# IuvenisSapiens/Qwen3-TTS-Rust

Hardware: AMD Instinct MI355X
Metric: audio-seconds generated per second (aggregate over GPUs) = concurrent real-time streams; RTF and first-chunk latency from the single-utterance leg (higher is better)
Workload: dtype i8

## Files before the change

### include/q3tts.h

```cpp
#ifndef Q3TTS_H
#define Q3TTS_H
#include <stdint.h>
#include <stddef.h>
#include "q3tts_spec.h"
#ifdef __cplusplus
extern "C" {
#endif

#define Q3TTS_OK 0
#define Q3TTS_ERR -1

const char* q3tts_last_error(void);
int q3tts_version(void);
int q3tts_device_count(void);

typedef struct q3tts_sampler_config {
    float temperature;
    int32_t top_k;
    float top_p;
    int32_t has_seed;
    uint64_t seed;
} q3tts_sampler_config;
void q3tts_sampler_config_default(q3tts_sampler_config* c);

// ... 309 lines not shown
                       uint16_t* ad);
int q3tts_op_matmul_float(const void* w , int32_t type, int32_t n, int32_t k, int32_t row0, int32_t nrows,
                          const float* x , int32_t ntok, float* y );
int q3tts_op_rmsnorm_quant(const float* x, const float* g, int32_t d, int32_t ntok, float eps, int8_t* xq, uint16_t* xd,
                           float* xn);
int q3tts_op_swiglu_quant(const float* gu, int32_t ff, int32_t ntok, int8_t* aq, uint16_t* ad);
int q3tts_op_argmax(const float* logits, int32_t n, int32_t start, int32_t end, int32_t mask_idx, int32_t* out);
int q3tts_op_sample(const float* logits, int32_t n, float temperature, int32_t top_k, float top_p, uint64_t seed, int32_t mask_idx,
                    int32_t n_draws, int32_t* out);
int q3tts_op_sample_rows(int32_t kernel, const float* logits, int32_t B, int32_t n, const float* temperature, const int32_t* top_k,
                         const float* top_p, const float* penalty, const uint64_t* seed, const int32_t* hist, const int32_t* hist_len,
                         int32_t hist_cap, int32_t n_draws, int32_t* out);
int q3tts_op_project(const float* x, const float* w , const float* b, int32_t n_in, int32_t n_out, float* y);
int q3tts_op_logprob_rows(const float* logits, int32_t B, int32_t n, int32_t stride, const int32_t* chosen, int32_t extra_idx,
                          float* out_chosen, float* out_extra);
int q3tts_op_score_rows(const float* tlogits, int32_t t_stride, const float* plogits, const int32_t* codes, int32_t F, float* out);
int q3tts_op_score_inputs(const float* hidden_proj, const float* const* tabs, const int64_t* tab_rows, int32_t dP, const int32_t* codes,
                          int32_t F, float* out);
int q3tts_op_kv_fork(uint16_t* k_cache, uint16_t* v_cache, int32_t n_pages, int32_t n_layer, int32_t n_kv, const int32_t* page_table,
                     int32_t n_seq, int32_t max_pages, int32_t src_seq, const int32_t* dst_seqs, int32_t n_dst, int32_t n_positions);
int q3tts_op_feedback_rows(const q3tts_assets* a, const int32_t* codes, int32_t n, const int32_t* trail_ids, int32_t n_trail, float* rows);
enum { Q3TTS_GEMM_AUTO = 0, Q3TTS_GEMM_SKINNY4 = 1, Q3TTS_GEMM_SKINNY8 = 2, Q3TTS_GEMM_SKINNY16 = 3,
       Q3TTS_GEMM_F32_1 = 4, Q3TTS_GEMM_F32_2 = 5,
       Q3TTS_GEMM_H1 = 6, Q3TTS_GEMM_H1_EPL = 7, Q3TTS_GEMM_H2 = 8, Q3TTS_GEMM_H2_EPL = 9,
       Q3TTS_GEMM_H3 = 10, Q3TTS_GEMM_H3_EPL = 11 };
enum { Q3TTS_EPI_NONE = 0, Q3TTS_EPI_GELU = 1, Q3TTS_EPI_RES_SCALE = 2 , Q3TTS_EPI_RES = 3 ,
       Q3TTS_EPI_SNAKE = 4  };
typedef struct q3tts_codec_gemm_desc {
    int32_t M, N, cin, taps, dil;
    const float* A; int64_t a_rows; int32_t lda, a_segT, a_skip;
    int32_t a_split, o_split;
    const float* W; const float* bias;
    int32_t epi; const float* res; int64_t res_floats; int32_t ldr, r_segT; int64_t r_skip;
    const float* scale; const float* snake_ea; const float* snake_ib;
    float* out; int64_t out_floats, out_off; int32_t ldo, o_segT; int64_t o_skip;
    int64_t ws_floats;
    int32_t form, ksplit, reducer;
    int32_t form_ran, ksplit_ran, reducer_ran;
} q3tts_codec_gemm_desc;
int q3tts_op_codec_gemm(q3tts_codec_gemm_desc* d);
int q3tts_codec_gemm_plan(q3tts_codec_gemm_desc* d);

enum { Q3TTS_CK_RVQ_SUM = 0, Q3TTS_CK_RMSNORM_ROWS = 1, Q3TTS_CK_LAYERNORM_ROWS = 2, Q3TTS_CK_ROPE_APPEND = 3, Q3TTS_CK_WINDOW_ATTN = 4,
       Q3TTS_CK_SWIGLU_ROWS = 5, Q3TTS_CK_DWCONV7 = 6, Q3TTS_CK_SNAKE = 7, Q3TTS_CK_SNAKE_SPLIT = 8, Q3TTS_CK_CONV_OUT_WAVE = 9,
       Q3TTS_CK_CONV_OUT_WIN = 10, Q3TTS_CK_HIST_LOAD = 11, Q3TTS_CK_HIST_SAVE = 12, Q3TTS_CK_HIST_ZERO = 13 };
typedef struct q3tts_codec_kernel_desc {
    int32_t kernel;
    int32_t G, T, C, H;
    int32_t n_heads, head_dim, window; float rope_base, eps, bias;
    const int64_t* meta;
    const int64_t* codes; int32_t n_q, cb_size;
    int32_t n_streams, stream;
    const float* in[3]; int64_t in_floats[3];
    const float* p0; const float* p1; int64_t p0_floats, p1_floats;
    float* out[3]; int64_t out_floats[3];
} q3tts_codec_kernel_desc;
int q3tts_op_codec_kernel(q3tts_codec_kernel_desc* d);

enum { Q3TTS_ATTN_AUTO = 0, Q3TTS_ATTN_UNFUSED = 1 , Q3TTS_ATTN_FUSED = 2 ,
       Q3TTS_ATTN_SHORT1 = 3, Q3TTS_ATTN_SHORT2 = 4 , Q3TTS_ATTN_GGML = 5  };
typedef struct q3tts_attention_desc {
    int32_t n_head, n_kv, n_layer, layer, ntok;
    const float* qkv; int32_t qkv_stride;
    const float* q_norm; const float* k_norm;
    float eps, rope_base; int32_t n_ctx; int32_t mrope_sec[4];
    const int32_t* seq; const int32_t* slot; const int32_t* pos; int32_t uniform_pos;
    const int32_t* page_table; int32_t n_seq, max_pages;
    uint16_t* k_cache; uint16_t* v_cache; int32_t n_pages;
    int32_t fused, fused_max_tok, same_seq, short_attn_min, hpw1_max, float_mode, ggml_mode;
    int32_t form;
    float* att; int8_t* aq; uint16_t* ad;
    int32_t form_ran;
} q3tts_attention_desc;
int q3tts_op_attention(q3tts_attention_desc* d);
int q3tts_op_attention_keyed(q3tts_attention_desc* d, const uint64_t* keys, int32_t key_stride, int32_t qkv_rows);
int q3tts_attention_plan(q3tts_attention_desc* d);

enum { Q3TTS_LOP_GEMV = 0, Q3TTS_LOP_GATEUP = 1, Q3TTS_LOP_NORM = 2, Q3TTS_LOP_NORM_GEMV = 3, Q3TTS_LOP_NORM_ARGMAX = 4, Q3TTS_LOP_NORM_GATEUP = 5,
       Q3TTS_LOP_F_GEMV = 6, Q3TTS_LOP_F_GATEUP = 7 };
enum { Q3TTS_LIN_AUTO = 0, Q3TTS_LIN_GEMV_Q8 = 1, Q3TTS_LIN_GEMM_Q8_TOK = 2, Q3TTS_LIN_GEMM_Q8_MFMA = 3, Q3TTS_LIN_GEMM_Q8_TILE1 = 4,
       Q3TTS_LIN_GEMV_KQ = 5, Q3TTS_LIN_GEMM_KQ_MFMA = 6, Q3TTS_LIN_GU_Q8_TILE1 = 7, Q3TTS_LIN_GU_Q8_MFMA = 8, Q3TTS_LIN_GU_KQ_MFMA = 9,
       Q3TTS_LIN_GU_UNFUSED = 10, Q3TTS_LIN_NORM = 11, Q3TTS_LIN_NORM_WG = 12, Q3TTS_LIN_GEMV_NORM = 13, Q3TTS_LIN_GEMV_NORM_ARGMAX = 14,
       Q3TTS_LIN_GU_SWIGLU_NORM = 15, Q3TTS_LIN_F_GEMV = 16, Q3TTS_LIN_F_MFMA16 = 17, Q3TTS_LIN_F_MFMA = 18, Q3TTS_LIN_F_GU_MFMA16 = 19,
       Q3TTS_LIN_F_GU_UNFUSED = 20 };
typedef struct q3tts_linear_desc {
    int32_t op, form;
    int32_t nw; const void* raw[3]; int32_t type[3]; int32_t rows[3]; int32_t kq_layout;
    int32_t K, row0, nrows, nrows_valid, ntok, ff;
    int32_t lpr, mt, ztiles;
    int32_t fused;
    const int8_t* xq; const uint16_t* xd; int32_t a_rows;
    const float* x; int64_t x_floats; int32_t x_off, x_stride;
    const float* h_in; int64_t h_floats; int32_t h_stride;
    const uint64_t* idx_keys; const int32_t* idx; int32_t idx_stride;
    const float* parts; int64_t parts_floats; int32_t nparts, parts_stride; int64_t parts_slab;
    const float* g; float eps;
    float* h_out; float* xn_out;
    int8_t* xq_out; uint16_t* xd_out;
    uint64_t* keys; int64_t n_keys; int32_t key_stride; const int32_t* mask_per_tok; int32_t idx_add;
    float* out; int64_t out_floats, out_off; int32_t out_stride;
    int8_t* aq; uint16_t* ad;
    int32_t form_ran, lpr_ran, mt_ran, z_ran;
} q3tts_linear_desc;
int q3tts_op_linear(q3tts_linear_desc* d);
int q3tts_linear_plan(q3tts_linear_desc* d);
uint64_t q3tts_argmax_key(float v, int32_t idx);

enum { Q3TTS_SEL_SAMPLE = 0, Q3TTS_SEL_SAMPLE_PRED = 1, Q3TTS_SEL_ARGMAX = 2, Q3TTS_SEL_ARGMAX_KEYS = 3 };
#define Q3TTS_SELECT_SENTINEL 0xA5C3F00D5A3C0FF1ull
typedef struct q3tts_select_desc {
    int32_t kernel;
    int32_t B, n, stride, row_off;
    const float* logits;
    const float* temperature; const int32_t* top_k; const float* top_p;
    const int32_t* mask_idx;
    const uint64_t* seed;
    const uint32_t* draw0;
    int32_t n_draws;
    const float* penalty; const int32_t* hist; const int32_t* hist_len; int32_t hist_cap; const int32_t* cur_code;
    int32_t out_stride;
    int32_t start, end, add;
    int32_t* tokens;
    uint64_t* out_raw;
    uint32_t* draws_out;
} q3tts_select_desc;
int q3tts_op_select_rows(q3tts_select_desc* d);

enum { Q3TTS_GLUE_PROJECT_MT = 0, Q3TTS_GLUE_PROJECT_TABLE = 1, Q3TTS_GLUE_FEEDBACK_KEYS = 2, Q3TTS_GLUE_GATHER_ROWS_KEYS = 3,
       Q3TTS_GLUE_ADVANCE_KEYS = 4, Q3TTS_GLUE_STALL_SAVE = 5, Q3TTS_GLUE_ADVANCE_KEYS_GATED = 6 };
#define Q3TTS_GLUE_GUARD 64
typedef struct q3tts_guarded { void* p; int64_t n; } q3tts_guarded;
typedef struct q3tts_frame_glue_desc {
    int32_t kernel;
    int32_t ntok;
    int32_t n_in, n_out, x_stride, x_off, out_stride;
    const float* x; int64_t x_floats;
    const float* w; const float* b;
    const float* const* tables; const int64_t* table_rows;
    int32_t row_len, key_stride;
    const float* tts_pad;
    int32_t trail; const int32_t* trail_ids; int32_t ids_stride; const float* text_table; int64_t text_rows;
    const int32_t* n_trail; const int32_t* open; const int32_t* max_frames;
    int32_t hist_stride;
    q3tts_guarded out;
    q3tts_guarded keys, next_key0;
    q3tts_guarded finished, n_frames, t_slot, t_pos, hist;
    q3tts_guarded hidden, save_hidden;
    q3tts_guarded draws, pdraws, save_draws;
} q3tts_frame_glue_desc;
int q3tts_op_frame_glue(q3tts_frame_glue_desc* d);

int q3tts_pcm_out_plan(int32_t rate, int32_t* L, int32_t* M, int32_t* n_taps, int32_t* taps_per_phase);
int64_t q3tts_pcm_out_filter(int32_t rate, float* h32, int64_t cap);
int64_t q3tts_pcm_out_samples(int32_t rate, int64_t n_native);
int q3tts_pcm_format_check(const q3tts_pcm_format* f);
int q3tts_op_pcm_convert(const float* in, int32_t G, const int32_t* chunk_samples, int32_t n_chunks, const int32_t* streams, int32_t n_streams,
                         const q3tts_pcm_format* fmt, const int32_t* reset_before, void* const* out, const int64_t* out_bytes, int64_t* n_out,
                         float* hist_store);

int64_t q3tts_tsm_samples(int32_t rate_pct, int64_t n_native, int32_t final);
int q3tts_tsm_windows(float* w, float* w2);
int q3tts_op_tsm(const float* in, int32_t G, const int32_t* chunk_samples, int32_t n_chunks, const int32_t* streams, int32_t n_streams,
                 const int32_t* rate_pct, const int32_t* encoding, const int32_t* reset_before, int32_t flush, void* const* out,
                 const int64_t* out_bytes, int64_t* n_out, int32_t* const* delta_trace, const int64_t* trace_len, float* hist_store);

#ifdef __cplusplus
}
// ... 3 lines not shown
```

### qwen3-tts-rust_amd/csrc/capi_ops.cpp

```cpp
#include "../../include/q3tts.h"
#include "transformer.h"
#include "host_logic.h"
#include "kdev.h"
#include "codec.h"
#include "kernels.h"
#include "pcm_out.h"
#include "tsm.h"

using namespace q3;
#define Q3_API_BEGIN try {
#define Q3_API_END(failval) } catch (const std::exception& ex) { set_last_error(ex.what()); return failval; } catch (...) { set_last_error("unknown error"); return failval; }
static void require_gpu() {
    int n = 0;
    if (hipGetDeviceCount(&n) != hipSuccess || n <= 0) throw Error("no HIP device available: the HIP path is the only compute path (no CPU fallback)");
}

static int attention_op_plan(const q3tts_attention_desc& d) {
    AttnPlanIn a;
    a.ntok = d.ntok; a.fused = d.fused != 0; a.fused_max_tok = d.fused_max_tok; a.same_seq = d.same_seq != 0; a.short_attn_min = d.short_attn_min;
    a.n_head = d.n_head; a.n_kv = d.n_kv; a.hpw1_max = d.hpw1_max > 0 ? d.hpw1_max : short_attn_hpw1_max();
    a.float_mode = d.float_mode != 0; a.ggml_mode = d.ggml_mode != 0;
    return plan_attention(a);
}

// ... 43 lines not shown
        }
        dkeys.alloc((size_t)(nt - 1) * key_stride + 1); dkeys.upload((const q3_u64*)keys, dkeys.n);
    }
    DevBuf<float> qkv((size_t)(keys ? qkv_rows : nt) * qs); qkv.upload(d.qkv, qkv.n);
    const QkvRows rows(qkv.p, qs, dkeys.p, key_stride);
    DevBuf<float> qn(128), kn(128); qn.upload(d.q_norm, 128); kn.upload(d.k_norm, 128);
    std::vector<float> hc, hs;
    build_rope_tables(d.rope_base, d.n_ctx, hc, hs);
    DevBuf<float> rc(hc.size()), rs(hs.size()); rc.upload(hc.data(), hc.size()); rs.upload(hs.data(), hs.size());
    DevBuf<int32_t> sec(4); sec.upload(d.mrope_sec, 4);
    DevBuf<int32_t> dseq, dslot, dpos, dtab;
    TokMeta tm{nullptr, nullptr, nullptr};
    if (d.uniform_pos >= 0) tm.uniform_pos = d.uniform_pos;
    else {
        dseq.alloc(nt); dseq.upload(d.seq, nt); dslot.alloc(nt); dslot.upload(d.slot, nt); dpos.alloc((size_t)nt * 4); dpos.upload(d.pos, (size_t)nt * 4);
        tm.seq = dseq.p; tm.slot = dslot.p; tm.pos = dpos.p;
    }
    const size_t cache_halfs = (size_t)d.n_pages * d.n_layer * d.n_kv * 8192;
    DevBuf<uint16_t> kc(cache_halfs), vc(cache_halfs);
    kc.upload(d.k_cache, cache_halfs); vc.upload(d.v_cache, cache_halfs);
    KvCache kv;
    kv.k = kc.p; kv.v = vc.p; kv.page_table = nullptr; kv.max_pages = d.page_table ? d.max_pages : 1; kv.n_layer = d.n_layer; kv.n_kv = d.n_kv;
    if (d.page_table) { dtab.alloc((size_t)d.n_seq * d.max_pages); dtab.upload(d.page_table, dtab.n); kv.page_table = dtab.p; }
    DevBuf<float> att((size_t)nt * dq), qrot, scores;
    DevBuf<int8_t> aq((size_t)nt * dq); DevBuf<uint16_t> ad((size_t)nt * (dq / 32));
    switch (form) {
    case ATTN_UNFUSED:
        qrot.alloc((size_t)nt * dq);
        launch_qk_rope_append(0, rows, nullptr, d.n_head, d.n_kv, qn.p, kn.p, d.eps, rc.p, rs.p, d.n_ctx, sec.p, tm, kv, d.layer, qrot.p, nt);
        launch_attention(0, qrot.p, d.n_head, d.n_kv, tm, kv, d.layer, att.p, aq.p, ad.p, nt);
        break;
    case ATTN_FUSED:
        launch_attention_fused(0, rows, d.n_head, d.n_kv, qn.p, kn.p, d.eps, rc.p, rs.p, d.n_ctx, sec.p, tm, kv, d.layer, aq.p, ad.p, nt);
        break;
    case ATTN_SHORT1: case ATTN_SHORT2:
        launch_attention_short(0, form == ATTN_SHORT1 ? 1 : 2, rows, d.n_head, d.n_kv, qn.p, kn.p, d.eps, rc.p, rs.p, d.n_ctx, sec.p, tm, kv,
                               d.layer, aq.p, ad.p, nt, att.p);
        break;
    default:
        scores.alloc((size_t)nt * d.n_head * d.n_ctx);
        gg_qk_rope_append(0, qkv.p, qs, d.n_head, d.n_kv, qn.p, kn.p, d.eps, rc.p, rs.p, d.n_ctx, sec.p, tm, kv, d.layer, nt);
        gg_attention(0, qkv.p, qs, d.n_head, d.n_kv, tm, kv, d.layer, att.p, scores.p, d.n_ctx, nt);
        break;
    }
    Q3_LAUNCH_CHECK();
    Q3_HIP(hipDeviceSynchronize());
    kc.download(d.k_cache, cache_halfs); vc.download(d.v_cache, cache_halfs);
    if (d.att && form != ATTN_FUSED) att.download(d.att, att.n);
    if (form != ATTN_GGML) { aq.download(d.aq, aq.n); ad.download(d.ad, ad.n); }
    if (keys) qkv.download(const_cast<float*>(d.qkv), qkv.n);
    d.form_ran = form;
}

static bool lin_quant(const q3tts_linear_desc& d) { return d.op <= LOP_NORM_GATEUP && d.op != LOP_NORM; }
static bool lin_kq(const q3tts_linear_desc& d) {
    if (d.kq_layout || d.nw > 1) return true;
    return d.type[0] != Q3_T_Q8_0;
}
static int lin_rows(const q3tts_linear_desc& d) { int n = 0; for (int i = 0; i < d.nw; i++) n += d.rows[i]; return n; }
static int lin_wts(const q3tts_linear_desc& d) {
    if (d.op >= LOP_F_GEMV) return d.type[0];
    if (!lin_kq(d)) return 0;
    int n = 0, last = -1;
    for (int i = 0; i < d.nw; i++) if (d.type[i] != last) { n++; last = d.type[i]; }
    return n == 1 ? d.type[0] : -1;
}
static LinearPlanIn lin_plan_in(const q3tts_linear_desc& d) {
    LinearPlanIn in;
    in.op = d.op; in.K = d.K; in.row0 = d.row0; in.nrows = d.nrows; in.ntok = d.ntok; in.ff = d.ff;
    in.kq = lin_quant(d) && lin_kq(d); in.wts = lin_wts(d); in.has_wt = true;
    if (in.kq) { int n = 0, last = -1; for (int i = 0; i < d.nw; i++) if (d.type[i] != last) { n++; last = d.type[i]; } in.kq_parts = n; }
    in.out_stride = d.out_stride; in.out_addr = (uintptr_t)d.out_off * 4 + (d.out ? (uintptr_t)d.out : 0);
    in.x_stride = d.x_stride; in.x_addr = (uintptr_t)d.x_off * 4 + (d.x ? (uintptr_t)d.x : 0);
    in.aq_addr = 0; in.fused = d.fused != 0;
    return in;
}
static LinearPlan lin_plan(const q3tts_linear_desc& d) {
    Q3_CHECK(d.op >= LOP_GEMV && d.op <= LOP_F_GATEUP, "unknown linear op");
    Q3_CHECK(d.K >= 256 && d.K % 256 == 0 && d.ntok >= 1 && d.ntok <= 65535 && d.nrows >= 1 && d.row0 >= 0, "bad linear shape");
    return plan_linear(lin_plan_in(d));
}
static bool in_set(int v, std::initializer_list<int> s) { for (int x : s) if (v == x) return true; return false; }
static int op_of_form(int f) {
    if (f <= LIN_GEMM_KQ_MFMA) return LOP_GEMV;
    if (f <= LIN_GU_UNFUSED) return LOP_GATEUP;
    if (f <= LIN_NORM_WG) return LOP_NORM;
    if (f == LIN_GEMV_NORM) return LOP_NORM_GEMV;
    if (f == LIN_GEMV_NORM_ARGMAX) return LOP_NORM_ARGMAX;
    if (f == LIN_GU_SWIGLU_NORM) return LOP_NORM_GATEUP;
    if (f <= LIN_F_MFMA) return LOP_F_GEMV;
    return LOP_F_GATEUP;
}
static void lin_check(const q3tts_linear_desc& d, const LinearPlan& p) {
    const int f = p.form, K = d.K, nt = d.ntok, ntiles = (nt + 31) / 32;
    Q3_CHECK(f >= LIN_GEMV_Q8 && f <= LIN_F_GU_UNFUSED && op_of_form(f) == d.op, "the form does not compute this op");
    const bool quant = lin_quant(d), kq = quant && lin_kq(d), norm = d.op >= LOP_NORM && d.op <= LOP_NORM_GATEUP;
    if (d.op != LOP_NORM) {
        Q3_CHECK(d.nw >= 1 && d.nw <= 3, "1 to 3 weight tensors");
        for (int i = 0; i < d.nw; i++) Q3_CHECK(d.raw[i] && d.rows[i] >= 1, "missing weight tensor");
        if (d.op >= LOP_F_GEMV) Q3_CHECK(d.nw == 1 && (d.type[0] == Q3_T_F32 || d.type[0] == Q3_T_F16 || d.type[0] == Q3_T_BF16), "float ops take one f32 / f16 / bf16 tensor");
        else if (kq) for (int i = 0; i < d.nw; i++) Q3_CHECK(in_set(d.type[i], {Q3_T_Q8_0, Q3_T_Q5_K, Q3_T_Q6_K}) && d.rows[i] % 32 == 0, "K-quant layout: Q8_0 / Q5_K / Q6_K tensors of 32-row multiples");
        Q3_CHECK(d.row0 + d.nrows <= lin_rows(d), "rows past the matrix");
    }
    if (d.op == LOP_GATEUP) Q3_CHECK(K <= 2048, "int8 gate/up: K <= 2048 (k_swiglu_quant reads one super-segment slab)");
    if (d.op == LOP_GATEUP || d.op == LOP_NORM_GATEUP || d.op == LOP_F_GATEUP)
        Q3_CHECK(d.row0 == 0 && d.nrows == 2 * d.ff && d.ff >= 1 && d.ff % (d.op == LOP_F_GATEUP ? 1 : 32) == 0, "gate/up: row0 0, nrows 2 * ff, ff % 32 == 0");
    if (quant && !norm) Q3_CHECK(d.xq && d.xd && d.a_rows >= nt, "int8 activations [a_rows >= ntok][K]");
    if (d.op >= LOP_F_GEMV) Q3_CHECK(d.x && d.x_off >= 0 && d.x_stride >= K && d.x_off + (int64_t)(nt - 1) * d.x_stride + K <= d.x_floats, "float activations out of their buffer");
    if (norm) {
        Q3_CHECK(K <= 2048 && d.h_in && d.g && d.h_stride >= K, "norm prologue: K <= 2048, h_in and g required");
        Q3_CHECK(!(d.idx && d.idx_keys), "idx or idx_keys, not both");
        if (d.idx) Q3_CHECK(f == LIN_NORM, "int32 row indices: NORM only");
        for (int t = 0; t < nt; t++) {
            int64_t row = t;
            if (d.idx) row = d.idx[(size_t)t * d.idx_stride];
            else if (d.idx_keys) row = key_code(d.idx_keys[(size_t)t * d.idx_stride]);
            Q3_CHECK(row >= 0 && row * d.h_stride + K <= d.h_floats, "selected h_in row outside h_in");
        }
        Q3_CHECK(d.nparts >= 0 && (d.nparts == 0 || (d.parts && d.parts_stride >= K && d.parts_slab >= 0 &&
                 (int64_t)(d.nparts - 1) * d.parts_slab + (int64_t)(nt - 1) * d.parts_stride + K <= d.parts_floats)), "residual slabs out of their buffer");
        if (f == LIN_NORM && d.nparts > 1) Q3_CHECK(d.parts_slab == (int64_t)nt * d.parts_stride, "NORM: slabs are ntok * parts_stride apart");
        if (d.op == LOP_NORM) Q3_CHECK(d.xq_out && d.xd_out, "NORM: xq_out / xd_out required");
    }
    if (in_set(d.op, {LOP_GEMV, LOP_NORM_GEMV, LOP_F_GEMV, LOP_F_GATEUP})) {
        const int64_t cols = d.op == LOP_F_GATEUP ? d.ff : d.nrows;
        const int64_t slabs = d.op == LOP_GEMV ? (K / 256 + 7) / 8 : 1;
        Q3_CHECK(d.out && d.out_off >= 0 && d.out_stride >= cols && d.out_off + (slabs * nt - 1) * d.out_stride + cols <= d.out_floats, "output out of its buffer");
    }
    if (in_set(d.op, {LOP_GATEUP, LOP_NORM_GATEUP})) Q3_CHECK(d.aq && d.ad, "gate/up: aq / ad required");
    if (f == LIN_GEMV_NORM_ARGMAX) {
        Q3_CHECK(d.keys && d.key_stride >= 1 && (int64_t)(nt - 1) * d.key_stride < d.n_keys, "argmax keys out of their buffer");
        Q3_CHECK(d.nrows_valid >= 1 && d.nrows_valid <= d.nrows, "1 <= nrows_valid <= nrows");
    }
    const bool q8 = quant && !kq;
    switch (f) {
    case LIN_GEMV_Q8: case LIN_GEMV_KQ:
        Q3_CHECK(f == LIN_GEMV_Q8 ? q8 : kq, "GEMV_Q8 takes the Q8_0 layout, GEMV_KQ the K-quant layout");
        Q3_CHECK(in_set(p.lpr, {2, 4, 8}) && in_set(p.mt, {1, 2, 4, 8}), "lpr in {2,4,8}, mt in {1,2,4,8}");
        break;
    case LIN_GEMM_Q8_TOK: Q3_CHECK(q8, "GEMM_Q8_TOK takes the Q8_0 layout"); break;
    case LIN_GEMM_Q8_MFMA: case LIN_GEMM_KQ_MFMA:
        Q3_CHECK(f == LIN_GEMM_Q8_MFMA ? q8 : kq, "GEMM_Q8_MFMA takes the Q8_0 layout, GEMM_KQ_MFMA the K-quant layout");
        Q3_CHECK(p.z >= 1 && p.z <= ntiles, "1 <= ztiles <= token tiles");
        break;
    case LIN_GEMM_Q8_TILE1:
        Q3_CHECK(q8 && K <= 1024 && d.nrows % 4 == 0 && d.out_stride % 4 == 0 && ((uintptr_t)(d.out + d.out_off) & 15) == 0 && p.z == ntiles,
                 "GEMM_Q8_TILE1: Q8_0, K <= 1024, nrows % 4 == 0, out_stride % 4 == 0, 16-byte out, ztiles == token tiles");
        break;
    case LIN_GU_Q8_TILE1: case LIN_GU_Q8_MFMA: case LIN_GU_KQ_MFMA:
        Q3_CHECK(f == LIN_GU_KQ_MFMA ? (kq && lin_wts(d) != -1) : q8, "GU_Q8_*: Q8_0 layout; GU_KQ_MFMA: K-quant layout of one tensor type");
        Q3_CHECK((K == 1024 || K == 2048) && d.ff % 32 == 0, "fused gate/up: K in {1024, 2048}, ff % 32 == 0");
        Q3_CHECK(p.z >= (ntiles + 3) / 4 && p.z <= ntiles && (f != LIN_GU_Q8_TILE1 || p.z == ntiles), "fused gate/up: ceil(tiles/4) <= ztiles <= tiles (TILE1: == tiles)");
        break;
    case LIN_GEMV_NORM: case LIN_GEMV_NORM_ARGMAX: case LIN_GU_SWIGLU_NORM:
        Q3_CHECK(f == LIN_GU_SWIGLU_NORM ? (in_set(p.mt, {1, 2, 4}) && lin_wts(d) != -1) : in_set(p.mt, {1, 2, 4, 8}), "mt out of range / GU_SWIGLU_NORM needs one tensor type");
        Q3_CHECK(f == LIN_GU_SWIGLU_NORM || (f == LIN_GEMV_NORM_ARGMAX ? p.lpr == 2 : in_set(p.lpr, {2, 4, 8})), "GEMV_NORM: lpr in {2,4,8}; ARGMAX: lpr 2");
        break;
    case LIN_F_GEMV: Q3_CHECK(in_set(p.mt, {1, 2, 4, 8}), "mt in {1,2,4,8}"); break;
    case LIN_F_MFMA16: case LIN_F_MFMA: case LIN_F_GU_MFMA16:
        Q3_CHECK(d.row0 % 64 == 0 && ((uintptr_t)(d.x + d.x_off) & 15) == 0 && d.x_stride % 4 == 0, "float matrix-core forms: row0 % 64 == 0, 16-byte x, x_stride % 4 == 0");
        if (f == LIN_F_GU_MFMA16) Q3_CHECK(d.ff % 16 == 0, "F_GU_MFMA16: ff % 16 == 0");
        break;
    default: break;
    }
}
static void lin_run(q3tts_linear_desc* dp) {
    Q3_CHECK(dp, "null linear descriptor");
    q3tts_linear_desc& d = *dp;
    LinearPlan p = lin_plan(d);
    if (d.form != LIN_AUTO) {
        Q3_CHECK(d.form >= LIN_GEMV_Q8 && d.form <= LIN_F_GU_UNFUSED, "unknown linear form");
        LinearPlan fp; fp.form = d.form; fp.nseg = d.K / 256;
        const int f = d.form, ntiles = (d.ntok + 31) / 32;
        const int mt_def = d.ntok == 1 ? 1 : d.ntok == 2 ? 2 : d.ntok <= 4 ? 4 : 8;
        fp.mt = d.mt ? d.mt : (p.form == f && p.mt ? p.mt : (f == LIN_GU_SWIGLU_NORM ? (mt_def > 4 ? 4 : mt_def) : mt_def));
        fp.lpr = d.lpr ? d.lpr : (p.form == f && p.lpr ? p.lpr : (f == LIN_GEMV_NORM_ARGMAX ? 2 : 8));
        int zdef = p.form == f && p.z ? p.z : ntiles;
        fp.z = d.ztiles ? d.ztiles : zdef;
        p = fp;
    }
    lin_check(d, p);
    const int K = d.K, nt = d.ntok, ff = d.ff;
    DevBuf<uint8_t> storage, fw, fwt;
    Q8Mat m; FMat fm;
    if (d.op >= LOP_F_GEMV) {
        const int n = d.rows[0];
        const size_t esz = d.type[0] == Q3_T_F32 ? 4 : 2;
        fw.alloc((size_t)n * K * esz); fw.upload((const uint8_t*)d.raw[0], fw.n);
        fwt.alloc((size_t)((n + 63) / 64) * 64 * K * esz);
        launch_tile_float(0, fw.p, fwt.p, d.type[0], n, K);
        fm.w = fw.p; fm.wt = fwt.p; fm.type = d.type[0]; fm.N = n; fm.K = K;
    } else if (d.op != LOP_NORM) {
        m = lin_kq(d) ? kqmat_from_host(d.raw, d.type, d.rows, d.nw, K, storage) : q8mat_from_host(d.raw[0], d.rows[0], K, storage);
    }
    DevBuf<int8_t> dxq; DevBuf<uint16_t> dxd; DevBuf<float> dx, dh, dparts, dg, dhout, dxn, dout, dgu;
    DevBuf<q3_u64> dkeys_in, dkeys; DevBuf<int32_t> didx, dmask; DevBuf<int8_t> daq, dxq_out; DevBuf<uint16_t> dad, dxd_out;
    if (d.xq) { dxq.alloc((size_t)d.a_rows * K); dxq.upload(d.xq, dxq.n); dxd.alloc((size_t)d.a_rows * (K / 32)); dxd.upload(d.xd, dxd.n); }
    if (d.op >= LOP_F_GEMV) { dx.alloc((size_t)d.x_floats); dx.upload(d.x, dx.n); }
    NormPro a{};
    const bool norm = d.op >= LOP_NORM && d.op <= LOP_NORM_GATEUP;
    if (norm) {
        dh.alloc((size_t)d.h_floats); dh.upload(d.h_in, dh.n);
        dg.alloc(K); dg.upload(d.g, K);
        a.h_in = dh.p; a.h_stride = d.h_stride; a.g = dg.p; a.eps = d.eps; a.idx_stride = d.idx_stride;
        if (d.idx_keys) { dkeys_in.alloc((size_t)(nt - 1) * d.idx_stride + 1); dkeys_in.upload((const q3_u64*)d.idx_keys, dkeys_in.n); a.idx_keys = dkeys_in.p; }
        if (d.idx) { didx.alloc((size_t)(nt - 1) * d.idx_stride + 1); didx.upload(d.idx, didx.n); }
        if (d.nparts > 0) { dparts.alloc((size_t)d.parts_floats); dparts.upload(d.parts, dparts.n); }
        a.parts = dparts.p; a.nparts = d.nparts; a.parts_stride = d.parts_stride; a.parts_slab = (size_t)d.parts_slab;
        if (d.h_out) { dhout.alloc((size_t)nt * K); dhout.upload(d.h_out, dhout.n); a.h_out = dhout.p; }
        if (d.xn_out) { dxn.alloc((size_t)nt * K); dxn.upload(d.xn_out, dxn.n); a.xn_out = dxn.p; }
    }
    if (d.out) { dout.alloc((size_t)d.out_floats); dout.upload(d.out, dout.n); }
    if (d.aq) { daq.alloc((size_t)nt * ff); daq.upload(d.aq, daq.n); dad.alloc((size_t)nt * (ff / 32)); dad.upload(d.ad, dad.n); }
    float* out = d.out ? dout.p + d.out_off : nullptr;
    switch (p.form) {
    case LIN_GEMV_Q8: case LIN_GEMM_Q8_TOK: case LIN_GEMM_Q8_MFMA: case LIN_GEMM_Q8_TILE1: case LIN_GEMV_KQ: case LIN_GEMM_KQ_MFMA:
        run_gemv_q8(0, p, m, d.row0, d.nrows, dxq.p, dxd.p, out, d.out_stride, nt);
        break;
    case LIN_GU_Q8_TILE1: case LIN_GU_Q8_MFMA: case LIN_GU_KQ_MFMA:
        run_gateup_q8(0, p, m, ff, dxq.p, dxd.p, daq.p, dad.p, nt);
        break;
    case LIN_GU_UNFUSED: {
        dgu.alloc((size_t)((K / 256 + 7) / 8) * nt * 2 * ff);
        LinearPlanIn gi = linear_plan_in(LOP_GEMV, m, 0, 2 * ff, nt);
        gi.out_stride = 2 * ff; gi.out_addr = (uintptr_t)dgu.p;
        const LinearPlan gp = plan_linear(gi);
        run_gemv_q8(0, gp, m, 0, 2 * ff, dxq.p, dxd.p, dgu.p, 2 * ff, nt);
        launch_swiglu_quant(0, dgu.p, ff, daq.p, dad.p, nt);
        p.lpr = gp.lpr; p.mt = gp.mt; p.z = gp.z;
        break;
    }
    case LIN_NORM: {
        dxq_out.alloc((size_t)nt * K); dxq_out.upload(d.xq_out, dxq_out.n); dxd_out.alloc((size_t)nt * (K / 32)); dxd_out.upload(d.xd_out, dxd_out.n);
        launch_rmsnorm_quant(0, norm_args(a, K, dxq_out.p, dxd_out.p, didx.p), nt);
        break;
    }
    case LIN_NORM_WG:
        dxq_out.alloc((size_t)nt * K); dxq_out.upload(d.xq_out, dxq_out.n); dxd_out.alloc((size_t)nt * (K / 32)); dxd_out.upload(d.xd_out, dxd_out.n);
        launch_rmsnorm_quant_wg(0, a, K, dxq_out.p, dxd_out.p, nt);
        break;
    case LIN_GEMV_NORM: case LIN_GEMV_NORM_ARGMAX: {
        ArgmaxEpi am{};
        if (p.form == LIN_GEMV_NORM_ARGMAX) {
            dkeys.alloc((size_t)d.n_keys); dkeys.upload((const q3_u64*)d.keys, dkeys.n);
            if (d.mask_per_tok) { dmask.alloc(nt); dmask.upload(d.mask_per_tok, nt); }
            am.keys = dkeys.p; am.key_stride = d.key_stride; am.mask_per_tok = dmask.p; am.idx_add = d.idx_add;
            run_gemv_q8_norm(0, p, m, d.row0, d.nrows_valid, a, nullptr, 0, nt, &am);
        } else run_gemv_q8_norm(0, p, m, d.row0, d.nrows, a, out, d.out_stride, nt, nullptr);
        break;
    }
    case LIN_GU_SWIGLU_NORM: run_gateup_swiglu(0, p, m, ff, a, daq.p, dad.p, nt); break;
    case LIN_F_GEMV: case LIN_F_MFMA16: case LIN_F_MFMA:
        run_gemv_float(0, p, fm, d.row0, d.nrows, dx.p + d.x_off, d.x_stride, out, d.out_stride, nt);
        break;
    case LIN_F_GU_MFMA16:
        dgu.alloc((size_t)nt * ff);
        run_gateup_float(0, p, fm, ff, dx.p + d.x_off, d.x_stride, dgu.p, nt);
        break;
    case LIN_F_GU_UNFUSED: {
        dgu.alloc((size_t)nt * 2 * ff);
        LinearPlanIn gi = lin_plan_in(d); gi.op = LOP_F_GEMV;
        const LinearPlan gp = plan_linear(gi);
        run_gemv_float(0, gp, fm, 0, 2 * ff, dx.p + d.x_off, d.x_stride, dgu.p, 2 * ff, nt);
        DevBuf<float> act((size_t)nt * ff);
        launch_swiglu_f32(0, dgu.p, ff, act.p, nt);
        Q3_HIP(hipMemcpy2D(out, (size_t)d.out_stride * 4, act.p, (size_t)ff * 4, (size_t)ff * 4, nt, hipMemcpyDeviceToDevice));
        Q3_HIP(hipDeviceSynchronize());
        p.lpr = gp.lpr; p.mt = gp.mt; p.z = gp.z;
        break;
    }
    default: throw Error("unhandled linear form");
    }
    Q3_LAUNCH_CHECK();
    if (p.form == LIN_F_GU_MFMA16) Q3_HIP(hipMemcpy2D(out, (size_t)d.out_stride * 4, dgu.p, (size_t)ff * 4, (size_t)ff * 4, nt, hipMemcpyDeviceToDevice));
    Q3_HIP(hipDeviceSynchronize());
    if (d.out) dout.download(d.out, dout.n);
    if (d.aq) { daq.download(d.aq, daq.n); dad.download(d.ad, dad.n); }
    if (d.h_out) dhout.download(d.h_out, dhout.n);
    if (d.xn_out) dxn.download(d.xn_out, dxn.n);
    if (dxq_out.p) { dxq_out.download(d.xq_out, dxq_out.n); dxd_out.download(d.xd_out, dxd_out.n); }
    if (dkeys.p) dkeys.download((q3_u64*)d.keys, dkeys.n);
    d.form_ran = p.form; d.lpr_ran = p.lpr; d.mt_ran = p.mt; d.z_ran = p.z;
}

template <class T> struct GlueBuf {
    DevBuf<T> d; T* host = nullptr; size_t n = 0;
    void up(const q3tts_guarded& g, size_t core, const char* what) {
        Q3_CHECK(g.p && g.n >= (int64_t)(core + 2 * Q3TTS_GLUE_GUARD), std::string("guarded buffer too small or missing: ") + what);
        host = (T*)g.p; n = (size_t)g.n;
        d.alloc(n); d.upload(host, n);
    }
    T* p() const { return d.p + Q3TTS_GLUE_GUARD; }
    void down() { if (host) d.download(host, n); }
};

extern "C" {

int q3tts_op_attention(q3tts_attention_desc* d) {
    Q3_API_BEGIN
    require_gpu();
    attention_op_run(d);
    return Q3TTS_OK;
    Q3_API_END(Q3TTS_ERR)
}

int q3tts_op_attention_keyed(q3tts_attention_desc* d, const uint64_t* keys, int32_t key_stride, int32_t qkv_rows) {
    Q3_API_BEGIN
    require_gpu();
    Q3_CHECK(keys, "null keys");
    attention_op_run(d, keys, key_stride, qkv_rows);
    return Q3TTS_OK;
    Q3_API_END(Q3TTS_ERR)
}

int q3tts_attention_plan(q3tts_attention_desc* d) {
    Q3_API_BEGIN
    Q3_CHECK(d && d->ntok >= 1 && d->n_kv >= 1 && d->n_head >= 1, "bad attention shape");
    d->form_ran = attention_op_plan(*d);
    return Q3TTS_OK;
    Q3_API_END(Q3TTS_ERR)
}

int q3tts_op_linear(q3tts_linear_desc* d) {
    Q3_API_BEGIN
    require_gpu();
    lin_run(d);
    return Q3TTS_OK;
    Q3_API_END(Q3TTS_ERR)
}

int q3tts_linear_plan(q3tts_linear_desc* d) {
    Q3_API_BEGIN
    Q3_CHECK(d, "null linear descriptor");
    const LinearPlan p = lin_plan(*d);
    d->form_ran = p.form; d->lpr_ran = p.lpr; d->mt_ran = p.mt; d->z_ran = p.z;
    return Q3TTS_OK;
    Q3_API_END(Q3TTS_ERR)
}

uint64_t q3tts_argmax_key(float v, int32_t idx) { return pack_key(v, idx); }

int q3tts_op_kv_fork(uint16_t* k_cache, uint16_t* v_cache, int32_t n_pages, int32_t n_layer, int32_t n_kv, const int32_t* page_table,
                     int32_t n_seq, int32_t max_pages, int32_t src_seq, const int32_t* dst_seqs, int32_t n_dst, int32_t n_positions) {
    Q3_API_BEGIN
    Q3_CHECK(k_cache && v_cache && page_table && dst_seqs, "null argument");
    Q3_CHECK(n_pages >= 1 && n_layer >= 1 && n_kv >= 1 && n_seq >= 1 && max_pages >= 1, "bad cache / page table shape");
    Q3_CHECK((int64_t)n_layer * n_kv <= 65536 && (int64_t)n_pages * n_layer * n_kv <= ((int64_t)1 << 24), "cache too large for the test surface");
    Q3_CHECK(n_dst >= 1, "n_dst must be >= 1");
    Q3_CHECK(n_positions >= 1 && (int64_t)n_positions <= (int64_t)max_pages * 64, "n_positions must be in [1, max_pages * 64]");
    Q3_CHECK(src_seq >= 0 && src_seq < n_seq, "source sequence out of range");
    const int np = (n_positions + 63) / 64;
    std::vector<int> owner((size_t)n_pages, -1);
    std::vector<char> listed((size_t)n_seq, 0);
    listed[src_seq] = 1;
    for (int d = -1; d < n_dst; d++) {
        const int seq = d < 0 ? src_seq : dst_seqs[d];
        if (d >= 0) {
            Q3_CHECK(seq >= 0 && seq < n_seq, "destination sequence out of range");
            Q3_CHECK(seq != src_seq, "a destination equals the source");
            Q3_CHECK(!listed[seq], "a destination is listed twice");
// ... 939 lines not shown
```

### qwen3-tts-rust_amd/csrc/engine.cpp

```cpp
#include "engine.h"
#include "../../include/q3tts.h"
#include <algorithm>
#include <cmath>
#include <chrono>
#include "kdev.h"
#include <functional>

namespace q3 {

static std::string quant_dir(const std::string& q) {
    if (q == "q5_k_m") return "gguf_q5_k_m";
    if (q == "q8_0") return "gguf_q8_0";
    if (q == "bf16") return "gguf_bf16";
    if (q == "f16") return "gguf_f16";
    return "gguf";
}
static double now_ms() {
    return std::chrono::duration<double, std::milli>(std::chrono::steady_clock::now().time_since_epoch()).count();
}

Engine::Engine(const EngineParams& p) : p_(p) {
    Q3_CHECK(p.max_batch >= 1 && p.max_batch <= 512, "max_batch out of range");
    Q3_HIP(hipGetDevice(&dev_));
    Q3_HIP(hipStreamCreateWithFlags(&st_, hipStreamNonBlocking));
    const std::string dir = p.model_dir + "/" + quant_dir(p.quant);
    assets_.reset(new HostAssets(dir + "/qwen3_assets.gguf"));
    const int B = p.max_batch;
    B_ = B;
    talker_.reset(new Transformer(dir + "/qwen3_tts_talker.gguf", Q3_TALKER_NCTX, std::max(256, B)));
    predictor_.reset(new Transformer(dir + "/qwen3_tts_predictor.gguf", Q3_PRED_NCTX, 2 * B));
    if (const char* e = std::getenv("Q3_PRED_FUSED_MAX")) predictor_->set_fused_max_tokens(atoi(e));
    {
        int min_tok = 8;
        if (const char* e = std::getenv("Q3_SHORT_ATTN_MIN")) min_tok = atoi(e);
        predictor_->set_short_attention(min_tok, 17);
    }
    Q3_CHECK(talker_->hp().n_embd == Q3_EMBD, "talker n_embd must be 2048 (reference hard-codes 2048-wide rows)");
    dP_ = predictor_->hp().n_embd;
    Q3_CHECK(assets_->proj_out == dP_ && assets_->proj_in == Q3_EMBD, "proj shape does not match predictor n_embd");
    Q3_CHECK(assets_->n_codec == 16, "need 16 codec embedding tables");
    Q3_CHECK(predictor_->hp().n_vocab >= 15 * Q3_CODEBOOK_SIZE, "predictor vocab < 15*2048");
    Q3_CHECK(dP_ % 16 == 0, "projection width must be a multiple of 16");
    {
        const std::vector<float> wt = project_wt(assets_->proj_w, Q3_EMBD, dP_), wb = project_wblk(assets_->proj_w, Q3_EMBD, dP_);
        d_proj_wt_.alloc(wt.size()); d_proj_wt_.upload(wt.data(), wt.size());
        d_proj_wblk_.alloc(wb.size()); d_proj_wblk_.upload(wb.data(), wb.size());
    }
    d_proj_b_.alloc(dP_); d_proj_b_.upload(assets_->proj_b, dP_);
    d_tts_pad_.alloc(Q3_EMBD); d_tts_pad_.upload(assets_->tts_pad(), Q3_EMBD);
    std::vector<const float*> ptrs(16);
    std::vector<int64_t> rows(16);
    for (int q = 0; q < 16; q++) {
        const size_t n = (size_t)assets_->codec_rows[q] * Q3_EMBD;
        d_codec_tab_[q].alloc(n); d_codec_tab_[q].upload(assets_->codec[q], n);
        d_proj_tab_[q].alloc((size_t)assets_->codec_rows[q] * dP_);
        launch_project_table(st_, d_codec_tab_[q].p, assets_->codec_rows[q], d_proj_wt_.p, d_proj_b_.p, Q3_EMBD, dP_, d_proj_tab_[q].p);
        ptrs[q] = d_codec_tab_[q].p; rows[q] = assets_->codec_rows[q];
    }
    d_tab_ptrs_.alloc(16); d_tab_ptrs_.upload(ptrs.data(), 16);
    d_tab_rows_.alloc(16); d_tab_rows_.upload(rows.data(), 16);
    pred_l0_table_ = !predictor_->ggml_mode();
    if (const char* e = std::getenv("Q3_PRED_L0_TABLE")) if (e[0] == '0') pred_l0_table_ = false;
    if (pred_l0_table_) {
        const int qs = (predictor_->hp().n_head + 2 * predictor_->hp().n_kv) * 128;
        Transformer wide(*predictor_, 256);
        for (int q = 1; q < 15; q++) {
            d_qkv0_tab_[q].alloc((size_t)assets_->codec_rows[q] * qs);
            wide.build_layer0_qkv(st_, d_proj_tab_[q].p, dP_, assets_->codec_rows[q], d_qkv0_tab_[q].p);
            pred_table_bytes_ += d_qkv0_tab_[q].n * sizeof(float);
        }
        Q3_HIP(hipStreamSynchronize(st_));
    }
    const int pages_per_seq = (p.max_prompt + p.max_steps + 1 + 63) / 64;
    kv_rows_ = (int64_t)pages_per_seq * 64;
    kv_t_.reset(new KvPool(talker_->hp().n_layer, talker_->hp().n_kv, B * pages_per_seq + 1, B + 1, pages_per_seq));
    kv_p_.reset(new KvPool(predictor_->hp().n_layer, predictor_->hp().n_kv, B, B, 1));
    for (int b = 0; b < B; b++) kv_p_->ensure(b, 16);
    pred_identity_pages_ = true;
    for (int b = 0; b < B; b++) if (kv_p_->page(b, 0) != b) pred_identity_pages_ = false;
    if (const char* e = std::getenv("Q3_UNIFORM_META")) if (e[0] == '0') pred_identity_pages_ = false;
    kv_t_->ensure(B, 1);
    {
        const char* e = std::getenv("Q3_ASYNC_PREFILL");
        async_pf_ = B > 1 && !(e && e[0] == '0');
    }
    if (async_pf_) {
        talker_pf_.reset(new Transformer(*talker_, 256));
        Q3_HIP(hipStreamCreateWithFlags(&st_pf_, hipStreamNonBlocking));
        Q3_HIP(hipEventCreate(&pf_done_)); Q3_HIP(hipEventCreate(&pf_e0_));
        lane_alloc(pf_, talker_pf_.get(), st_pf_, 256, true, (size_t)4096 * (Q3_EMBD * 4 + 24 + 68 + 64) + ((size_t)1 << 16) + (size_t)B * 4);
    }
    hist_stride_ = p.max_steps * 16;
    tl_stride_ = (Q3_SAMPLE_END + 31) & ~31;
    slots_ = SlotTable(B); d_slots_.alloc(slots_.host.size()); slots_.dev = d_slots_.p;
    d_keys_.alloc(16 * B); d_next_key0_.alloc(B); d_hist_.alloc((size_t)B * hist_stride_);
    d_rngkey_.alloc((size_t)8 * B); d_draws_.alloc(B); d_prngkey_.alloc((size_t)8 * B); d_pdraws_.alloc(B);
    d_rngkey_.zero(); d_draws_.zero(); d_prngkey_.zero(); d_pdraws_.zero(); d_plogits_.alloc((size_t)B * Q3_CODEBOOK_SIZE);
    d_tlogits_.alloc((size_t)B * tl_stride_); d_thidden_.alloc((size_t)B * Q3_EMBD); d_pin_.alloc((size_t)2 * B * dP_);
    d_fb_.alloc((size_t)B * Q3_EMBD);
    d_hist_.zero(); d_tlogits_.zero(); d_thidden_.zero();
    std::vector<int32_t> seq(B), slot((size_t)16 * B), pos((size_t)16 * B * 4);
    for (int b = 0; b < B; b++) {
        seq[b] = b;
        for (int i = 0; i < 16; i++) { slot[(size_t)i * B + b] = i; for (int s = 0; s < 4; s++) pos[((size_t)i * B + b) * 4 + s] = i; }
    }
    d_pseq_.alloc(B); d_pseq_.upload(seq.data(), B);
    d_pslot_.alloc(slot.size()); d_pslot_.upload(slot.data(), slot.size());
    d_ppos_.alloc(pos.size()); d_ppos_.upload(pos.data(), pos.size());
    h_pend_.assign(B, std::vector<int32_t>()); h_pend_off_.assign(B, 0);
    slot_req_.assign(B, nullptr);
    if (const char* e = std::getenv("Q3_SCORE_WIDTH")) score_w_ = std::max(16, std::min(64, atoi(e)));
    if (async_pf_) { d_pf_logits_.alloc((size_t)B * tl_stride_); d_pf_hidden_.alloc((size_t)B * Q3_EMBD); }
    {
        std::vector<q3_u64> k0((size_t)16 * B, pack_key(-INFINITY, 0)), n0(B, pack_key(-INFINITY, 0));
        d_keys_.upload(k0.data(), k0.size()); d_next_key0_.upload(n0.data(), n0.size());
    }
    lane_alloc(ar_, talker_.get(), st_, talker_->max_tok(), false, (size_t)talker_->max_tok() * Q3_EMBD * 4 + (size_t)B * 4096 + ((size_t)1 << 20));
    Q3_HIP(hipDeviceSynchronize());
    upload_slot_state();
    if (p.load_codec) {
        Q3_CHECK(p.max_steps <= Q3TTS_CODEC_MAX_FRAMES, "max_steps above Q3TTS_CODEC_MAX_FRAMES: a request's codec stream could not be decoded to its end");
        static const int group_env = [] { const char* e = std::getenv("Q3_CODEC_GROUP"); return e ? atoi(e) : 0; }();
        const int group_cap = group_env > 0 ? group_env : (B >= 128 ? 32 : 16);
        const int n_cs = B + std::min(B, 16), gmax = std::max(1, std::min(B, group_cap));
        static const int lanes_env = [] { const char* e = std::getenv("Q3_CODEC_LANES"); return e ? atoi(e) : 0; }();
        const int n_lanes = B > 1 ? (lanes_env > 0 ? std::min(lanes_env, 8) : 2) : 1;
        codec_.reset(new CodecDecoder(p.model_dir + "/onnx/q3tts_codec.gguf", n_cs, 4, n_lanes, gmax));
        st2_.resize(n_lanes);
        for (auto& s2 : st2_) Q3_HIP(hipStreamCreateWithFlags(&s2, hipStreamNonBlocking));
        slot_cap_ = (size_t)p.max_steps * codec_->samples_per_frame();
        Q3_HIP(hipHostMalloc((void**)&pcm_pinned_, (size_t)n_cs * slot_cap_ * sizeof(float)));
        Q3_HIP(hipHostMalloc((void**)&pre_tails_, (size_t)Q3TTS_MAX_PREAMBLES * Q3_PCM_HIST * sizeof(float)));
        for (int i = Q3TTS_MAX_PREAMBLES - 1; i >= 0; i--) pre_tail_free_.push_back(i);
        for (int c = n_cs - 1; c >= 0; c--) cs_free_.push_back(c);
        decode_w_ = q3::decode_width(n_cs, B);
    }
    Q3_HIP(hipStreamSynchronize(st_));
    Q3_HIP(hipDeviceSynchronize());
    ar_.cur.reset();
}

void Engine::lane_alloc(PrefillLane& L, Transformer* talker, hipStream_t st, int chunk, bool async, size_t arena_bytes) {
    L.talker = talker; L.st = st; L.chunk = chunk; L.async = async;
    L.d_rows.alloc((size_t)chunk * Q3_EMBD); L.d_seq.alloc(chunk); L.d_slot.alloc(chunk); L.d_pos.alloc(4 * (size_t)chunk);
    L.d_codes.alloc((size_t)chunk * 16); L.d_ids.alloc(chunk); L.d_fork_dst.alloc(B_);
    L.cur.cap = arena_bytes;
    Q3_HIP(hipHostMalloc((void**)&L.arena, arena_bytes));
}
void* Engine::stage_take(PrefillLane& L, size_t bytes) {
    size_t at = L.cur.take(bytes);
    if (at == StageCursor::NONE) {
        Q3_CHECK(!L.async, "prefill staging arena overflow");
        Q3_HIP(hipStreamSynchronize(L.st));
        L.cur.reset();
        at = L.cur.take(bytes);
        Q3_CHECK(at != StageCursor::NONE, "staging request larger than the arena");
    }
    return L.arena + at;
}
void Engine::h2d(void* dst, const void* src, size_t bytes) {
    void* p = stage_alloc(bytes);
    std::memcpy(p, src, bytes);
    Q3_HIP(hipMemcpyAsync(dst, p, bytes, hipMemcpyHostToDevice, st_));
}
void* Engine::d2h_begin(const void* src, size_t bytes) {
    void* p = stage_alloc(bytes);
    Q3_HIP(hipMemcpyAsync(p, src, bytes, hipMemcpyDeviceToHost, st_));
    return p;
}

struct CandSet { std::vector<float> prompt; std::vector<int32_t> trail; };
struct Engine::Req {
    int64_t id = 0;
// ... 851 lines not shown
    q3_u64 armed[17]; std::fill_n(armed, 17, pack_key(-INFINITY, 0));
    bool prefix_pcm = false;
    for (Req* r : batch) prefix_pcm = prefix_pcm || (r->want_pcm && r->r.n_prefix >= 4);
    {
        DecHold hold(this, codec_ != nullptr && prefix_pcm);
        for (Req* r : batch) {
            const int b = r->slot;
            slots_.load(b, r->r);
            const int k = r->r.n_prefix;
            const uint32_t draws = r->r.sampler.temperature > 0.0f ? (uint32_t)k : 0u, pdraws = 15u * (uint32_t)k;
            if (k > 0) {
                h2d(d_hist_.p + (size_t)b * hist_stride_, r->prefix_own.data(), (size_t)k * 64);
                push_frames(*r->chunker, r->prefix_own.data(), k);
            }
            StdRng rng(r->seed);
            h2d(d_rngkey_.p + (size_t)b * 8, rng.key(), 32);
            h2d(d_draws_.p + b, &draws, 4);
            if (r->r.opts.pred_sampled()) {
                StdRng prng(r->seed ^ (uint64_t)Q3_PRED_SEED_XOR);
                h2d(d_prngkey_.p + (size_t)b * 8, prng.key(), 32);
                h2d(d_pdraws_.p + b, &pdraws, 4);
            }
            h_pend_[b].clear();
            std::vector<int32_t> ids;
            { std::lock_guard<std::mutex> lk(mu_); ids = r->trail_ids(); slots_.hi(SF_OPEN)[b] = r->r.open && !r->closed; }
            slots_.hi(SF_NTRAIL)[b] = (int)ids.size();
            if (!ids.empty()) h2d(d_trail_.p + (size_t)b * p_.max_prompt, ids.data(), ids.size() * 4);
            h2d(d_keys_.p + (size_t)b * 16, armed, 16 * 8);
            h2d(d_next_key0_.p + b, armed, 8);
            if (lp_ready_.load()) {
                const int32_t rec = r->r.logprobs ? 1 : 0;
                h2d(d_lp_rec_.p + b, &rec, 4);
                if (rec) Q3_HIP(hipMemsetD32Async((hipDeviceptr_t)(d_lp_.p + (size_t)b * lp_rows_ * Q3_LOGPROB_COLS), (int)q3_f32_bits(Q3_LOGPROB_NONE),
                                                  (size_t)lp_rows_ * Q3_LOGPROB_COLS, st_));
            }
            slots_.live[b] = 1;
        }
    }
    upload_slot_state();
}

void Engine::activate() {
    std::vector<Req*> batch, dropped, scores;
    batch.swap(pf_batch_);
    {
        std::lock_guard<std::mutex> lk(mu_);
        const double t = now_ms();
        for (Req* r : batch) if (r->cancel) { r->prefill_ms = t - r->t_submit; dropped.push_back(r); }
        batch.erase(std::remove_if(batch.begin(), batch.end(), [](Req* r) { return r->cancel; }), batch.end());
    }
    for (Req* r : dropped) retire(r, false);
    for (Req* r : batch) if (r->score) scores.push_back(r);
    batch.erase(std::remove_if(batch.begin(), batch.end(), [](Req* r) { return r->score; }), batch.end());
    go_live(batch);
    for (Req* r : batch) {
        const int b = r->slot;
        Q3_HIP(hipMemcpyAsync(d_thidden_.p + (size_t)b * Q3_EMBD, d_pf_hidden_.p + (size_t)b * Q3_EMBD, (size_t)Q3_EMBD * 4, hipMemcpyDeviceToDevice, st_));
        SampleArgs sa = first_head_args(d_pf_logits_.p + (size_t)b * tl_stride_, b);
        if (resumed_penalised(r->r)) head_history(sa, b);
        launch_sample(st_, sa, 1);
        if (r->r.logprobs) first_head_logprobs(st_, d_pf_logits_.p + (size_t)b * tl_stride_, b, r->r.n_prefix);
    }
    Q3_HIP(hipStreamSynchronize(st_));
    { float ms = 0; Q3_HIP(hipEventElapsedTime(&ms, pf_e0_, pf_done_)); stats.prefill_ms += ms; }
    n_prefilling_ = 0;
    {
        const double t = now_ms();
        std::lock_guard<std::mutex> lk(mu_);
        for (Req* r : batch) r->prefill_ms = t - r->t_submit;
        for (Req* r : scores) r->prefill_ms = t - r->t_submit;
        n_active_ += (int)batch.size();
    }
    finish_scores(scores);
}

void Engine::ensure_score() {
    std::lock_guard<std::mutex> lk(sc_mu_);
    if (sc_ready_.load()) return;
    std::lock_guard<std::mutex> cap(capture_mutex());
    int prev = 0;
    Q3_HIP(hipGetDevice(&prev));
    Q3_HIP(hipSetDevice(dev_));
    try {
        const int W = score_w_, rows = std::max(talker_->max_tok(), 256);
        pred_sc_.reset(new Transformer(*predictor_, 16 * W));
        kv_sc_.reset(new KvPool(predictor_->hp().n_layer, predictor_->hp().n_kv, W, W, 1));
        for (int w = 0; w < W; w++) kv_sc_->ensure(w, 16);
        std::vector<int32_t> seq, slot, pos;
        for (int F = 1; F <= W; F++)
            for (int p = 0; p < 16; p++)
                for (int f = 0; f < F; f++) { seq.push_back(f); slot.push_back(p); for (int s4 = 0; s4 < 4; s4++) pos.push_back(p); }
        d_sc_seq_.alloc(seq.size()); d_sc_seq_.upload(seq.data(), seq.size());
        d_sc_slot_.alloc(slot.size()); d_sc_slot_.upload(slot.data(), slot.size());
        d_sc_pos_.alloc(pos.size()); d_sc_pos_.upload(pos.data(), pos.size());
        std::vector<const float*> tabs(15); std::vector<int64_t> tab_rows(15);
        for (int q = 0; q < 15; q++) { tabs[q] = d_proj_tab_[q].p; tab_rows[q] = assets_->codec_rows[q]; }
        d_sc_tabs_.alloc(15); d_sc_tabs_.upload(tabs.data(), 15);
        d_sc_tab_rows_.alloc(15); d_sc_tab_rows_.upload(tab_rows.data(), 15);
        d_sc_codes_.alloc((size_t)rows * 16); d_sc_tlogits_.alloc((size_t)rows * tl_stride_); d_sc_hidden_.alloc((size_t)rows * Q3_EMBD);
        d_sc_hproj_.alloc((size_t)W * dP_); d_sc_in_.alloc((size_t)16 * W * dP_); d_sc_plogits_.alloc((size_t)15 * W * Q3_CODEBOOK_SIZE);
        d_sc_out_.alloc((size_t)B_ * p_.max_steps * Q3_LOGPROB_COLS);
        Q3_HIP(hipStreamSynchronize(nullptr));
    } catch (...) { (void)hipSetDevice(prev); throw; }
    Q3_HIP(hipSetDevice(prev));
    sc_ready_ = true;
}

int64_t Engine::submit_score(const float* prompt, int n_prompt, const int32_t* trail, int n_trail, const int32_t* codes, int n) {
    if (const char* why = score_refusal(prompt, n_prompt, p_.max_prompt, trail, n_trail, codes, n, p_.max_steps, kv_rows_, talker_->ggml_mode()))
        throw Error(why);
    ensure_score();
    if (n_trail > 0) ensure_text_stream();
    std::unique_ptr<Req> r(new Req());
    r->score = true;
    GenRequest& g = r->r;
    g.n_prompt = n_prompt; g.max_steps = n; g.sampler.temperature = 0.0f; g.n_trail = n_trail;
    g.n_prefix = n - 1;
    r->prompt_own.assign(prompt, prompt + (size_t)n_prompt * Q3_EMBD); g.prompt = r->prompt_own.data();
    r->trail_own.assign(trail, trail + n_trail); g.trail = r->trail_own.data();
    r->prefix_own.assign(codes, codes + (size_t)n * 16); g.prefix = r->prefix_own.data();
    r->t_submit = now_ms();
    std::lock_guard<std::mutex> lk(mu_);
    return enqueue(std::move(r), pending_);
}

void Engine::score_chunk(hipStream_t st, Transformer& talker, const std::vector<Req*>& batch, const std::vector<ScoreRun>& runs, int32_t* h_codes) {
    if (runs.empty()) return;
    const int W = score_w_;
    int at = 0;
    for (const ScoreRun& run : runs) {
        Req* r = batch[run.req];
        Q3_CHECK((size_t)(at + run.n) * 16 <= d_sc_codes_.n && run.frame + run.n <= r->r.max_steps, "score rows outside the chunk buffers");
        std::copy(r->prefix_own.begin() + (size_t)run.frame * 16, r->prefix_own.begin() + (size_t)(run.frame + run.n) * 16, h_codes + (size_t)at * 16);
        Q3_HIP(hipMemcpyAsync(d_sc_codes_.p + (size_t)at * 16, h_codes + (size_t)at * 16, (size_t)run.n * 64, hipMemcpyHostToDevice, st));
        talker.head(st, run.row, run.n, 0, tl_stride_, d_sc_tlogits_.p + (size_t)at * tl_stride_, tl_stride_, nullptr, -1, d_sc_hidden_.p + (size_t)at * Q3_EMBD);
        for (int f0 = 0; f0 < run.n; f0 += W) {
            const int F = std::min(W, run.n - f0);
            const int32_t* codes = d_sc_codes_.p + (size_t)(at + f0) * 16;
            launch_project_blk(st, d_sc_hidden_.p + (size_t)(at + f0) * Q3_EMBD, Q3_EMBD, d_proj_wblk_.p, d_proj_b_.p, Q3_EMBD, dP_, d_sc_hproj_.p, dP_, F);
            launch_score_inputs(st, d_sc_hproj_.p, d_sc_tabs_.p, d_sc_tab_rows_.p, dP_, codes, F, d_sc_in_.p);
            const size_t m0 = (size_t)16 * F * (F - 1) / 2;
            TokMeta tm{d_sc_seq_.p + m0, d_sc_slot_.p + m0, d_sc_pos_.p + m0 * 4};
            Transformer::Input in; in.x = d_sc_in_.p; in.x_stride = dP_;
            pred_sc_->set_same_seq_tokens(true);
            pred_sc_->forward(st, in, 16 * F, tm, kv_sc_->view(), nullptr);
            for (int q = 0; q < 15; q++)
                pred_sc_->head(st, (q + 1) * F, F, q * Q3_CODEBOOK_SIZE, Q3_CODEBOOK_SIZE, d_sc_plogits_.p + (size_t)q * W * Q3_CODEBOOK_SIZE, Q3_CODEBOOK_SIZE);
            ScoreRowsArgs sa;
            sa.tlogits = d_sc_tlogits_.p + (size_t)(at + f0) * tl_stride_; sa.t_stride = tl_stride_;
            sa.plogits = d_sc_plogits_.p; sa.p_head_stride = (size_t)W * Q3_CODEBOOK_SIZE; sa.codes = codes;
            sa.out = d_sc_out_.p + ((size_t)r->slot * p_.max_steps + run.frame + f0) * Q3_LOGPROB_COLS;
            launch_score_rows(st, sa, F);
        }
        at += run.n;
    }
    Q3_LAUNCH_CHECK();
}

void Engine::finish_scores(const std::vector<Req*>& scores) {
    for (Req* r : scores) {
        const int b = r->slot, n = r->r.max_steps;
        bool cancelled;
        { std::lock_guard<std::mutex> lk(mu_); cancelled = r->cancel; }
        const float* rows = nullptr;
        if (!cancelled) {
            ar_.cur.reset();
            rows = (const float*)d2h_begin(d_sc_out_.p + (size_t)b * p_.max_steps * Q3_LOGPROB_COLS, (size_t)n * Q3_LOGPROB_COLS * 4);
// ... 451 lines not shown
```

### qwen3-tts-rust_amd/csrc/engine.h

```cpp
#pragma once
#include "transformer.h"
#include "host_logic.h"
#include "sched_logic.h"
#include "codec.h"
#include <atomic>
#include <condition_variable>
#include <deque>
#include <map>
#include <memory>
#include <mutex>
#include <thread>

namespace q3 {

struct EngineParams {
    std::string model_dir;
    std::string quant = "q8_0";
    int max_batch = 1;
    int max_prompt = 1024;
    int max_steps = Q3_DEFAULT_MAX_STEPS;
    bool load_codec = true;
    bool use_graph = true;
};

// ... 75 lines not shown
    int register_voice(const Voice& v);
    const Voice& voice(int id) const;

    const HostAssets& assets() const { return *assets_; }
    Transformer& talker() { return *talker_; }
    Transformer& predictor() { return *predictor_; }
    CodecDecoder* codec() { return codec_.get(); }
    EngineStats stats; void reset_stats() { stats = EngineStats(); }
    void set_instrument(bool on) { instrument_ = on; }
    size_t bytes_per_frame_step(int batch, double mean_ctx) const;
    size_t pred_table_bytes() const { return pred_table_bytes_; }
    hipStream_t stream() const { return st_; }
    int max_batch() const { return B_; }
    int device() const { return dev_; }

private:
    struct Req;
    struct FrameGraph {
        int width = 0; hipGraph_t graph = nullptr; hipGraphExec_t exec = nullptr;
        DevBuf<int32_t> seqA, slotA, posA;
    };
    void record_frame(FrameGraph& fg, FrameVariant v);
    FrameGraph& frame_graph(int width, FrameVariant v, bool capture);
    void validate(const GenRequest& g) const;
    void ensure_text_stream();
    Req& req(int64_t id);
    int64_t enqueue(std::unique_ptr<Req> r, std::deque<Req*>& queue);
    struct PrefillLane {
        Transformer* talker = nullptr; hipStream_t st = nullptr; int chunk = 0; bool async = false;
        DevBuf<float> d_rows; DevBuf<int32_t> d_seq, d_slot, d_pos;
        DevBuf<int32_t> d_codes, d_ids, d_fork_dst;
        unsigned char* arena = nullptr; StageCursor cur;
    };
    void lane_alloc(PrefillLane& L, Transformer* talker, hipStream_t st, int chunk, bool async, size_t arena_bytes);
    void* stage_take(PrefillLane& L, size_t bytes);
    void prefill_wave(PrefillLane& L, const std::vector<Req*>& wave, bool sampled);
    void head_live(Req* lead, const std::vector<Req*>& rest, int tok, bool sampled);
    void head_staged(Req* lead, const std::vector<Req*>& rest, int tok);
    SampleArgs first_head_args(const float* logits_row, int b) const;
    void feedback_rows(hipStream_t st, const std::vector<Req*>& batch, const std::vector<FbRun>& fb, int32_t* hc, int32_t* d_codes, int32_t* d_ids, float* d_rows);
    void head_history(SampleArgs& sa, int b) const;
    static bool resumed_penalised(const GenRequest& g) { return g.n_prefix > 0 && g.opts.penalised(); }
    void first_head_logprobs(hipStream_t st, const float* logits_row, int b, int row);
    void ensure_score();
    void score_chunk(hipStream_t st, Transformer& talker, const std::vector<Req*>& batch, const std::vector<ScoreRun>& runs, int32_t* h_codes);
    void finish_scores(const std::vector<Req*>& scores);
    static void split_sets(const std::vector<Req*>& batch, std::vector<Req*>& lead, std::vector<std::vector<Req*>>& rest);
    void fork_sets(hipStream_t st, const std::vector<Req*>& lead, const std::vector<std::vector<Req*>>& rest, int32_t* h_dst, int32_t* d_dst);
    static int kv_positions(const GenRequest& g, bool score) { return score ? g.n_prompt + g.n_prefix + 1 : g.n_prompt + g.max_steps + 1; }
    void prefill_async(const std::vector<Req*>& wave);
    void go_live(const std::vector<Req*>& batch);
    void activate();
    void admit_decodes();
    void enqueue_decodes();
    void admit(bool stalled);
    void run_group();
    void collect_appends();
    void collect_cancels();
    void harvest(bool block);
    void purge_chunks(Req* r);
    void retire(Req* r, bool flush_tail);
    void decoder_main();
    int64_t copy_pcm(const Req& r, void* out, int64_t off, int64_t cap) const;
    static int64_t pack_fmt(const q3tts_pcm_format& f) { return (int64_t)f.sample_rate * 4 + f.encoding; }
    static q3tts_pcm_format unpack_fmt(int64_t v) { return q3tts_pcm_format{(int32_t)(v / 4), (int32_t)(v % 4)}; }
    std::atomic<int64_t> out_fmt_{(int64_t)Q3_PCM_NATIVE_RATE * 4 + Q3_PCM_F32};
    std::atomic<int> rate_pct_{100};
    void take_rate(Req* r, int max_steps, int given = -1) const;
    void upload_slot_state();
    void* stage_alloc(size_t bytes) { return stage_take(ar_, bytes); }
    void h2d(void* dst, const void* src, size_t bytes);
    void* d2h_begin(const void* src, size_t bytes);

    EngineParams p_;
    hipStream_t st_ = nullptr; int dev_ = 0;
    std::vector<hipStream_t> st2_;
    float* pcm_pinned_ = nullptr; size_t slot_cap_ = 0;
    unsigned char* pcm_stage(const Req& r, size_t add) const;
    std::unique_ptr<HostAssets> assets_;
    std::unique_ptr<Transformer> talker_, predictor_, talker_pf_;
    hipStream_t st_pf_ = nullptr; PrefillLane ar_, pf_;
    DevBuf<float> d_pf_logits_, d_pf_hidden_;
    std::vector<Req*> pf_batch_; hipEvent_t pf_done_ = nullptr, pf_e0_ = nullptr; bool async_pf_ = false; int n_prefilling_ = 0;
    std::unique_ptr<KvPool> kv_t_, kv_p_;
    std::unique_ptr<CodecDecoder> codec_;
    DevBuf<float> d_codec_tab_[16]; DevBuf<float> d_proj_tab_[16];
    DevBuf<float> d_qkv0_tab_[16]; bool pred_l0_table_ = false; size_t pred_table_bytes_ = 0;
    DevBuf<float> d_proj_wt_, d_proj_wblk_, d_proj_b_, d_tts_pad_;
    DevBuf<const float*> d_tab_ptrs_; DevBuf<int64_t> d_tab_rows_;
    int dP_ = 0;
    int B_ = 0; SlotTable slots_; DevBuf<uint32_t> d_slots_; bool slot_dirty_ = false;
    int32_t* di(SlotField f) const { return slots_.di(f); } float* df(SlotField f) const { return slots_.df(f); }
    DevBuf<int32_t> d_hist_; DevBuf<q3_u64> d_keys_, d_next_key0_;
    DevBuf<uint32_t> d_rngkey_, d_draws_, d_prngkey_, d_pdraws_; DevBuf<float> d_plogits_;
    DevBuf<int32_t> d_pseq_, d_pslot_, d_ppos_;
    DevBuf<float> d_tlogits_, d_thidden_, d_pin_, d_fb_;
    int64_t kv_rows_ = 0;
    int hist_stride_ = 0, tl_stride_ = 0;
    DevBuf<float> d_text_; DevBuf<int32_t> d_trail_; int64_t text_rows_ = 0;
    std::mutex text_mu_; bool text_ready_ = false;
    DevBuf<float> d_stall_hidden_; DevBuf<uint32_t> d_stall_draws_;
    DevBuf<float> d_lp_, d_plp_; DevBuf<int32_t> d_lp_rec_; int lp_rows_ = 0;
    std::mutex lp_mu_; std::atomic<bool> lp_on_{false}, lp_ready_{false};
    std::unique_ptr<Transformer> pred_sc_; std::unique_ptr<KvPool> kv_sc_; int score_w_ = 32;
    DevBuf<int32_t> d_sc_seq_, d_sc_slot_, d_sc_pos_, d_sc_codes_; DevBuf<const float*> d_sc_tabs_; DevBuf<int64_t> d_sc_tab_rows_;
    DevBuf<float> d_sc_tlogits_, d_sc_hidden_, d_sc_hproj_, d_sc_in_, d_sc_plogits_, d_sc_out_;
    std::mutex sc_mu_; std::atomic<bool> sc_ready_{false};
    int64_t next_set_ = 1;
    std::atomic<int64_t> cand_sets_{0}, cand_rows_saved_{0}, cand_pages_{0};
    std::map<int, std::unique_ptr<FrameGraph>> graphs_;
    bool instrument_ = false; bool pred_identity_pages_ = false;
    std::vector<std::vector<int32_t>> h_pend_; std::vector<int> h_pend_off_;
    std::mutex mu_; std::condition_variable cv_;
    std::mutex step_mu_;
    std::map<int64_t, std::unique_ptr<Req>> reqs_;
    std::deque<Req*> pending_;
    std::vector<Req*> slot_req_;
    std::vector<int> cs_free_;
    int64_t next_id_ = 1;
    int n_active_ = 0, n_draining_ = 0;
    std::deque<Req*> decode_q_; int n_decoding_ = 0, decode_w_ = 0;
    std::vector<Req*> dec_admitted_;
    std::atomic<int64_t> dec_reqs_{0}, dec_chunks_{0}, dec_shared_{0};
    struct Preamble { PreambleRefs refs; int n = 0, snap = -1, tail = -1; };
    std::map<int, Preamble> pres_; int next_pre_ = 0, eng_pre_ = -1;
    float* pre_tails_ = nullptr; std::vector<int> pre_tail_free_;
    std::atomic<int64_t> pre_built_{0}, pre_restores_{0};
    void pre_attach(Req* r, int pid);
    void pre_drop(Req* r);
    void pre_unhold(int pid);
    bool trail_dirty_ = false;
    std::vector<int64_t> cancel_ids_;
    uint64_t wake_ = 0;
    bool stalled_idle_ = false;
    std::vector<Voice> voices_;
    std::thread driver_; bool driver_on_ = false, driver_stop_ = false;
    struct DecTask { Req* r; std::vector<int64_t> codes; bool is_final; bool fence; bool reset; int64_t epoch = 0; };
    struct Completion { Req* r; hipEvent_t ev; size_t pcm_after; bool fence; };
    std::thread dec_thread_; bool dec_started_ = false, dec_stop_ = false;
    std::mutex dmu_; std::condition_variable dcv_;
    std::deque<DecTask> dq_, dq_lo_; std::deque<Completion> comp_;
    bool dec_hold_ = false;
    int64_t dec_epoch_ = 0;
    struct DecHold {
        Engine* e; bool on;
        DecHold(Engine* e_, bool on_) : e(e_), on(on_) { if (on) { e->dec_epoch_++; std::lock_guard<std::mutex> lk(e->dmu_); e->dec_hold_ = true; } }
        ~DecHold() { if (on) { { std::lock_guard<std::mutex> lk(e->dmu_); e->dec_hold_ = false; } e->dcv_.notify_all(); } }
    };
    int dec_pending_ = 0;
    std::string derr_;
    LaunchTimer timer_, timer_gu_;
};

}
```

### qwen3-tts-rust_amd/csrc/kernels.h

```cpp
#pragma once
#include <hip/hip_runtime.h>
#include <cstdint>
#include <vector>
#include "wlayout.h"
#include "q3_common.h"

namespace q3 {

struct Q8Mat {
    const uint8_t* qs = nullptr;
    const uint16_t* sc = nullptr;
    int N = 0;
    int Npad = 0;
    int K = 0;
    const uint8_t* rg_type = nullptr;
    const uint32_t* rg_off = nullptr;
    const uint8_t* meta = nullptr;
    size_t qbytes = 0;
    int nparts = 0; int p1_rg0 = 0x7fffffff, p2_rg0 = 0x7fffffff; int p0_type = 0, p1_type = 0, p2_type = 0; uint32_t p0_off = 0, p1_off = 0, p2_off = 0;
    size_t bytes() const { return (qbytes ? qbytes : (size_t)Npad * K) + (size_t)Npad * (K / 32) * 2 + (meta ? (size_t)Npad * (K / 256) * 16 : 0); }
};

struct TokMeta {
    const int32_t* seq;
// ... 41 lines not shown
    __device__ __forceinline__ const float* row(int tok) const {
        return base + (size_t)(keys ? (int)(~(uint32_t)keys[(size_t)tok * key_stride]) : tok) * stride;
    }
};

void launch_qk_rope_append(hipStream_t st, const QkvRows& qkv, const float* parts_unused, int n_head, int n_kv,
                           const float* q_norm_w, const float* k_norm_w, float eps, const float* rope_cos,
                           const float* rope_sin, int n_ctx, const int32_t* mrope_sec , const TokMeta& tm,
                           const KvCache& kv, int layer, float* qrot, int ntok);

void launch_attention(hipStream_t st, const float* qrot, int n_head, int n_kv, const TokMeta& tm, const KvCache& kv,
                      int layer, float* att , int8_t* aq, uint16_t* ad, int ntok);

void launch_swiglu_quant(hipStream_t st, const float* gu, int ff, int8_t* aq, uint16_t* ad, int ntok);

void launch_argmax(hipStream_t st, const float* logits, int stride, int start, int end, const int32_t* mask_per_tok,
                   int32_t* out, int out_stride, int add, int ntok);

inline std::vector<float> project_wt(const float* w, int n_in, int n_out) {
    std::vector<float> wt((size_t)n_in * n_out);
    for (int o = 0; o < n_out; o++)
        for (int i = 0; i < n_in; i++) wt[(size_t)i * n_out + o] = w[(size_t)o * n_in + i];
    return wt;
}
inline std::vector<float> project_wblk(const float* w, int n_in, int n_out) {
    std::vector<float> wb((size_t)((n_out + 15) / 16) * 16 * n_in, 0.0f);
    for (int o = 0; o < n_out; o++)
        for (int i = 0; i < n_in; i++) wb[((size_t)(o / 16) * n_in + i) * 16 + (o % 16)] = w[(size_t)o * n_in + i];
    return wb;
}
void launch_project_table(hipStream_t st, const float* table, int64_t rows, const float* Wt, const float* b, int n_in,
                          int n_out, float* out);

void launch_argmax_keys(hipStream_t st, const float* logits, int stride, int n, const int32_t* mask_per_tok, unsigned long long* keys,
                        int key_stride, int ntok);


void launch_copy_f32(hipStream_t st, const float* src, float* dst, size_t n);
void init_kernel_attributes();

struct FMat { const void* w = nullptr; const void* wt = nullptr; int type = 0; int N = 0, K = 0; size_t bytes() const { return (size_t)N * K * (type == 0 ? 4 : 2); } };
void launch_gemv_float(hipStream_t st, const FMat& w, int row0, int nrows, const float* x, int x_stride, float* out, int out_stride, int ntok);
bool launch_gateup_float(hipStream_t st, const FMat& wgu, int ff, const float* x, int x_stride, float* act, int ntok);
void launch_tile_float(hipStream_t st, const void* w, void* wt, int type, int N, int K);
void launch_swiglu_f32(hipStream_t st, const float* gu, int ff, float* out, int ntok);

typedef unsigned long long q3_u64;
struct NormPro {
    const float* h_in; int h_stride;
    const q3_u64* idx_keys; int idx_stride;
    const float* parts; int nparts; int parts_stride; size_t parts_slab;
    float* h_out;
    const float* g; float eps;
    float* xn_out;
};
struct ArgmaxEpi {
    q3_u64* keys; int key_stride;
    const int32_t* mask_per_tok;
    int idx_add;
};
void launch_gemv_q8_norm(hipStream_t st, const Q8Mat& w, int row0, int nrows, const NormPro& a, float* out, int out_stride,
                         int ntok, const ArgmaxEpi* am);
void launch_rmsnorm_quant_wg(hipStream_t st, const NormPro& a, int d, int8_t* xq, uint16_t* xd, int ntok);
inline NormArgs norm_args(const NormPro& p, int d, int8_t* xq, uint16_t* xd, const int32_t* idx = nullptr) {
    return NormArgs{p.h_in, p.h_stride, idx, p.idx_stride, p.idx_keys, p.parts, p.nparts, p.parts_stride, p.h_out, p.g, p.eps, d, xq, xd, p.xn_out};
}
void launch_gateup_swiglu(hipStream_t st, const Q8Mat& wgu, int ff, const NormPro& a, int8_t* aq, uint16_t* ad, int ntok);
void launch_attention_fused(hipStream_t st, const QkvRows& qkv, int n_head, int n_kv, const float* q_norm_w,
                            const float* k_norm_w, float eps, const float* rope_cos, const float* rope_sin, int n_ctx,
                            const int32_t* mrope_sec, const TokMeta& tm, const KvCache& kv, int layer, int8_t* aq, uint16_t* ad,
                            int ntok);
void launch_attention_short(hipStream_t st, int hpw, const QkvRows& qkv, int n_head, int n_kv, const float* q_norm_w,
                            const float* k_norm_w, float eps, const float* rope_cos, const float* rope_sin, int n_ctx,
                            const int32_t* mrope_sec, const TokMeta& tm, const KvCache& kv, int layer, int8_t* aq, uint16_t* ad, int ntok,
                            float* att = nullptr );
int short_attn_hpw1_max();
void launch_project_blk(hipStream_t st, const float* x, int x_stride, const float* Wblk , const float* b,
                        int n_in, int n_out, float* out, int out_stride, int ntok);
enum LinearOp { LOP_GEMV = 0, LOP_GATEUP = 1, LOP_NORM = 2, LOP_NORM_GEMV = 3, LOP_NORM_ARGMAX = 4, LOP_NORM_GATEUP = 5, LOP_F_GEMV = 6,
                LOP_F_GATEUP = 7 };
enum LinearForm { LIN_AUTO = 0, LIN_GEMV_Q8 = 1, LIN_GEMM_Q8_TOK = 2, LIN_GEMM_Q8_MFMA = 3, LIN_GEMM_Q8_TILE1 = 4, LIN_GEMV_KQ = 5,
                  LIN_GEMM_KQ_MFMA = 6, LIN_GU_Q8_TILE1 = 7, LIN_GU_Q8_MFMA = 8, LIN_GU_KQ_MFMA = 9, LIN_GU_UNFUSED = 10, LIN_NORM = 11,
                  LIN_NORM_WG = 12, LIN_GEMV_NORM = 13, LIN_GEMV_NORM_ARGMAX = 14, LIN_GU_SWIGLU_NORM = 15, LIN_F_GEMV = 16, LIN_F_MFMA16 = 17,
                  LIN_F_MFMA = 18, LIN_F_GU_MFMA16 = 19, LIN_F_GU_UNFUSED = 20 };
struct LinearPlanIn {
    int op = LOP_GEMV;
    int K = 0, row0 = 0, nrows = 0, ntok = 0, ff = 0;
    int wts = 0;
    bool kq = false;
    int kq_parts = 0;
    bool has_wt = false;
    int out_stride = 0; uintptr_t out_addr = 0;
    int x_stride = 0; uintptr_t x_addr = 0;
    uintptr_t aq_addr = 0;
    int lpr_hint = 0;
    bool fused = true;
};
struct LinearPlan { int form = LIN_AUTO, lpr = 0, mt = 0, z = 0, nseg = 0; };
LinearPlan plan_linear(const LinearPlanIn& in);
void run_gemv_q8(hipStream_t st, const LinearPlan& p, const Q8Mat& w, int row0, int nrows, const int8_t* xq, const uint16_t* xd, float* out,
                 int out_stride, int ntok);
void run_gateup_q8(hipStream_t st, const LinearPlan& p, const Q8Mat& wgu, int ff, const int8_t* xq, const uint16_t* xd, int8_t* aq, uint16_t* ad,
                   int ntok);
void run_gemv_q8_norm(hipStream_t st, const LinearPlan& p, const Q8Mat& w, int row0, int nrows, const NormPro& a, float* out, int out_stride,
                      int ntok, const ArgmaxEpi* am);
void run_gateup_swiglu(hipStream_t st, const LinearPlan& p, const Q8Mat& wgu, int ff, const NormPro& a, int8_t* aq, uint16_t* ad, int ntok);
void run_gemv_float(hipStream_t st, const LinearPlan& p, const FMat& w, int row0, int nrows, const float* x, int x_stride, float* out,
                    int out_stride, int ntok);
void run_gateup_float(hipStream_t st, const LinearPlan& p, const FMat& wgu, int ff, const float* x, int x_stride, float* act, int ntok);
LinearPlanIn linear_plan_in(int op, const Q8Mat& w, int row0, int nrows, int ntok);
struct TextTrail {
    const int32_t* n_frames = nullptr; const int32_t* n_trail = nullptr; const int32_t* ids = nullptr; int ids_stride = 0;
    const float* table = nullptr; int64_t rows = 0;
};
void launch_feedback_keys(hipStream_t st, const float* const* tables, const int64_t* table_rows, const q3_u64* keys, int key_stride,
                          const float* tts_pad, float* out, int ntok, const TextTrail* trail = nullptr);
struct FeedbackIds { const int32_t* ids = nullptr; int n_ids = 0; const float* table = nullptr; int64_t rows = 0; };
void launch_feedback_codes(hipStream_t st, const float* const* tables, const int64_t* table_rows, const int32_t* codes, const float* tts_pad,
                           float* out, int n, const FeedbackIds* ids = nullptr);
void launch_gather_rows_keys(hipStream_t st, const float* table, int64_t rows, const q3_u64* keys, int key_stride, int row_len,
                             float* dst, int ntok);
struct AdvanceKeysArgs {
    int B; int32_t *finished, *n_frames; const int32_t* max_frames; q3_u64* keys; q3_u64* next_key0; int32_t* hist; int hist_stride;
    int32_t *t_slot, *t_pos;
};
void launch_advance_keys(hipStream_t st, const AdvanceKeysArgs& a);
struct StallArgs {
    const int32_t* open = nullptr; const int32_t* n_trail = nullptr;
    float* hidden = nullptr; uint32_t* draws = nullptr; uint32_t* pdraws = nullptr;
    float* save_hidden = nullptr; uint32_t* save_draws = nullptr;
};
void launch_stall_save(hipStream_t st, const AdvanceKeysArgs& a, const StallArgs& s);
void launch_advance_keys_gated(hipStream_t st, const AdvanceKeysArgs& a, const StallArgs& s);

struct SampleArgs {
    const float* logits; int stride; int n;
    const float* temperature; const int32_t* top_k; const float* top_p;
    const int32_t* mask_idx;
    const uint32_t* rng_key; uint32_t* draws;
    q3_u64* out_key; int out_stride;
    const float* penalty = nullptr;
    const int32_t* hist = nullptr; int hist_stride = 0; const int32_t* hist_len = nullptr;
    const q3_u64* cur_key = nullptr; int cur_stride = 0;
};
void launch_sample(hipStream_t st, const SampleArgs& a, int B);
void launch_sample_pred(hipStream_t st, const SampleArgs& a, int B);

struct LogprobHead {
    const float* logits = nullptr; int stride = 0; size_t head_stride = 0; int n = 0;
    const q3_u64* key = nullptr; int key_stride = 0; const int32_t* chosen = nullptr;
    int extra_idx = -1; int col = 0, col_extra = -1; int row_ahead = 0;
};
struct LogprobArgs {
    LogprobHead p; int n_first = 0; LogprobHead t;
    float* out = nullptr; int out_stride = 0, out_rows = 0;
    const int32_t* n_frames = nullptr; const int32_t* finished = nullptr; const int32_t* max_frames = nullptr;
    const int32_t* open = nullptr; const int32_t* n_trail = nullptr; const int32_t* record = nullptr;
};
void launch_logprob_rows(hipStream_t st, const LogprobArgs& a, int B);

void launch_score_inputs(hipStream_t st, const float* hidden_proj, const float* const* tabs, const int64_t* tab_rows, int dP, const int32_t* codes,
                         int F, float* out);
struct ScoreRowsArgs {
    const float* tlogits = nullptr; int t_stride = 0;
    const float* plogits = nullptr; size_t p_head_stride = 0;
    const int32_t* codes = nullptr; float* out = nullptr;
};
// ... 53 lines not shown
```

### qwen3-tts-rust_amd/csrc/kernels.hip

```cpp
#include "kernels.h"
#include <cstdlib>
#include "q3_common.h"
#include "../../include/q3tts_spec.h"
#include "kdev.h"
#include "wslice.h"

namespace q3 {

Q3_STAMP_SETTER(set_stamp_buffer)

template <int LPR, int MT>
__global__ void __launch_bounds__(512) k_gemv_q8(Q8Mat w, int row0, int nrows, const int8_t* __restrict__ xq,
                                                 const uint16_t* __restrict__ xd, float* __restrict__ out,
                                                 int out_stride, int ntok) {
    constexpr int R = 64 / LPR, BPL = LPR / 2, NLD = 8 / BPL;
    __shared__ float red[8][R * MT];
    const int lane = threadIdx.x & 63, wave = threadIdx.x >> 6;
    const int r = lane % R, q = lane / R, half = q & 1, bil = q >> 1;
    const int nseg = w.K >> 8, nb = w.K >> 5;
    const int sseg = blockIdx.y, seg = sseg * 8 + wave;
    const int tok0 = blockIdx.z * MT;
    const bool active = seg < nseg;
    float acc[MT];
#pragma unroll
    for (int m = 0; m < MT; m++) acc[m] = 0.0f;
    if (active) {
        int row = row0 + blockIdx.x * R + r;
        if (row > w.Npad - 1) row = w.Npad - 1;
        const int rg = row >> 5, r32 = row & 31;
        const uint8_t* base = w.qs + ((size_t)rg * nb + (size_t)seg * 8) * 1024 + half * 512 + r32 * 16;
        uint4 wv[NLD];
#pragma unroll
        for (int i = 0; i < NLD; i++) wv[i] = *reinterpret_cast<const uint4*>(base + (size_t)(i * BPL + bil) * 1024);
        const uint4 dwv = *reinterpret_cast<const uint4*>(w.sc + (((size_t)rg * nseg + seg) * 32 + r32) * 8);
#pragma unroll
        for (int m = 0; m < MT; m++) {
            int tok = tok0 + m;
            if (tok > ntok - 1) tok = ntok - 1;
            const int8_t* xp = xq + (size_t)tok * w.K + seg * 256;
            const uint4 dxv = *reinterpret_cast<const uint4*>(xd + (size_t)tok * nb + seg * 8);
#pragma unroll
            for (int i = 0; i < NLD; i++) {
                const uint4 xv = *reinterpret_cast<const uint4*>(xp + (i * BPL + bil) * 32 + half * 16);
                int isum = dot16(wv[i], xv);
                isum += xor_lane<R>(isum);
#pragma unroll
                for (int j = 0; j < BPL; j++) {
                    const int isj = (BPL == 1) ? isum : __shfl(isum, r + 2 * j * R);
                    const int b = i * BPL + j;
                    const float sc = h2f(half_of(dwv, b)) * h2f(half_of(dxv, b));
                    acc[m] = q3_fmaf((float)isj, sc, acc[m]);
                }
            }
        }
        if (q == 0) {
#pragma unroll
            for (int m = 0; m < MT; m++) red[wave][m * R + r] = acc[m];
        }
    }
    wg_barrier_lds();
    for (int t = threadIdx.x; t < R * MT; t += blockDim.x) {
        const int m = t / R, rr = t % R;
        int nsg = nseg - sseg * 8;
        if (nsg > 8) nsg = 8;
        float v[8];
#pragma unroll
        for (int s = 0; s < 8; s++) v[s] = red[s][t];
        float S = v[0];
#pragma unroll
        for (int s = 1; s < 8; s++) S = (s < nsg) ? S + v[s] : S;
        const int orow = blockIdx.x * R + rr, tok = tok0 + m;
        if (orow < nrows && tok < ntok) out[((size_t)sseg * ntok + tok) * out_stride + orow] = S;
    }
}

__global__ void k_gemm_q8_tok(Q8Mat w, int row0, int nrows, const int8_t* __restrict__ xq, const uint16_t* __restrict__ xd,
                              float* __restrict__ out, int out_stride, int ntok);
#define Q3_GEMM_Q8_BUDGET __launch_bounds__(512) __attribute__((amdgpu_waves_per_eu(4, 4)))
template <bool GU>
__global__ void Q3_GEMM_Q8_BUDGET k_gemm_q8_mfma(Q8Mat w, int row0, int nrows, const int8_t* __restrict__ xq, const uint16_t* __restrict__ xd,
                               float* __restrict__ out, int out_stride, int ntok, int ff, int8_t* __restrict__ aq, uint16_t* __restrict__ ad);
template <bool GU>
__global__ void Q3_GEMM_Q8_BUDGET k_gemm_q8_tile1(Q8Mat w, int row0, int nrows, const int8_t* __restrict__ xq, const uint16_t* __restrict__ xd,
                               float* __restrict__ out, int out_stride, int ntok, int ff, int8_t* __restrict__ aq, uint16_t* __restrict__ ad);
template <int TYPE>
__global__ void __launch_bounds__(512) __attribute__((amdgpu_waves_per_eu(2, 2)))
k_gemm_float_mfma(const void* __restrict__ wt, int K, int tile0, int nrows, const float* __restrict__ x, int x_stride, float* __restrict__ out, int out_stride, int ntok);
void init_fused_kernel_attributes();
void init_kernel_attributes() {
    static bool done[64] = {};
    int dev = 0;
    Q3_HIP(hipGetDevice(&dev));
    if (dev < 0 || dev > 63 || done[dev]) return;
    Q3_HIP(hipFuncSetAttribute((const void*)k_gemm_q8_tok, hipFuncAttributeMaxDynamicSharedMemorySize, 160 * 1024));
    constexpr int lds = Q3_SSEG_SEGS * 64 * 33 * (int)sizeof(float);
    Q3_HIP(hipFuncSetAttribute(reinterpret_cast<const void*>(&k_gemm_float_mfma<Q3_T_F32>), hipFuncAttributeMaxDynamicSharedMemorySize, lds));
    Q3_HIP(hipFuncSetAttribute(reinterpret_cast<const void*>(&k_gemm_float_mfma<Q3_T_F16>), hipFuncAttributeMaxDynamicSharedMemorySize, lds));
    Q3_HIP(hipFuncSetAttribute(reinterpret_cast<const void*>(&k_gemm_float_mfma<Q3_T_BF16>), hipFuncAttributeMaxDynamicSharedMemorySize, lds));
    init_fused_kernel_attributes();
    done[dev] = true;
}
static bool kq_mfma() { static const bool on = [] { const char* e = std::getenv("Q3_KQ_MFMA"); return e ? e[0] == '1' : true; }(); return on; }
template <bool GU, int TS>
__global__ void __launch_bounds__(512) __attribute__((amdgpu_waves_per_eu(2, 2)))
k_gemm_kq_mfma(Q8Mat w, int row0, int nrows, const int8_t* __restrict__ xq, const uint16_t* __restrict__ xd, float* __restrict__ out, int out_stride,
               int ntok, int ff, int8_t* __restrict__ aq, uint16_t* __restrict__ ad);
static int mfma_ztiles(int rowgroups, int nsseg, int ntok) {
    const int ntiles = (ntok + 31) / 32;
    static const int target = [] { const char* e = std::getenv("Q3_MFMA_WGS"); return e ? atoi(e) : 1024; }();
    int z = (target + rowgroups * nsseg - 1) / (rowgroups * nsseg);
    return z < 1 ? 1 : (z > ntiles ? ntiles : z);
}

template <int LPR, int MT, int TS>
__global__ void __launch_bounds__(512) k_gemv_kq(Q8Mat w, int row0, int nrows, const int8_t* __restrict__ xq,
                                                 const uint16_t* __restrict__ xd, float* __restrict__ out, int out_stride, int ntok) {
    constexpr int R = 64 / LPR;
    __shared__ float red[8][R * MT];
    const int lane = threadIdx.x & 63, wave = threadIdx.x >> 6;
    const int r = lane % R, q = lane / R, half = q & 1, bil = q >> 1;
    const int nseg = w.K >> 8, nb = w.K >> 5;
    const int sseg = blockIdx.y, seg = sseg * 8 + wave;
    const int tok0 = blockIdx.z * MT;
    const bool active = seg < nseg;
    float acc[MT];
#pragma unroll
    for (int m = 0; m < MT; m++) acc[m] = 0.0f;
    if (active) {
        int row = row0 + blockIdx.x * R + r;
        if (row > w.Npad - 1) row = w.Npad - 1;
        wslice_dispatch<TS>(w, row >> 5, [&](auto tag) {
            WSlice<LPR, decltype(tag)::value> ws;
            ws.load(w, row >> 5, row & 31, seg, half, bil);
            ws.finish(half);
#pragma unroll
            for (int m = 0; m < MT; m++) {
                int tok = tok0 + m;
                if (tok > ntok - 1) tok = ntok - 1;
                const uint4 dxv = *reinterpret_cast<const uint4*>(xd + (size_t)tok * nb + seg * 8);
                acc[m] = ws.chain(acc[m], xq + (size_t)tok * w.K + seg * 256, dxv, r, half, bil);
            }
        });
        if (q == 0) {
#pragma unroll
            for (int m = 0; m < MT; m++) red[wave][m * R + r] = acc[m];
        }
    }
    wg_barrier_lds();
    for (int t = threadIdx.x; t < R * MT; t += blockDim.x) {
        const int m = t / R, rr = t % R;
        int nsg = nseg - sseg * 8;
        if (nsg > 8) nsg = 8;
        float v[8];
#pragma unroll
        for (int s = 0; s < 8; s++) v[s] = red[s][t];
        float S = v[0];
#pragma unroll
        for (int s = 1; s < 8; s++) S = (s < nsg) ? S + v[s] : S;
        const int orow = blockIdx.x * R + rr, tok = tok0 + m;
        if (orow < nrows && tok < ntok) out[((size_t)sseg * ntok + tok) * out_stride + orow] = S;
    }
}
template <int LPR>
static void gemv_kq_mt(hipStream_t st, int mt, const Q8Mat& w, int row0, int nrows, const int8_t* xq, const uint16_t* xd, float* out,
                       int out_stride, int ntok) {
    constexpr int R = 64 / LPR;
    const int nseg = w.K >> 8, nsseg = (nseg + 7) / 8, nw = nseg < 8 ? nseg : 8;
    dim3 grid((nrows + R - 1) / R, nsseg, (ntok + mt - 1) / mt);
    if (mt == 1) Q3_TS_SWITCH(w, hipLaunchKernelGGL((k_gemv_kq<LPR, 1, TS>), grid, dim3(64 * nw), 0, st, w, row0, nrows, xq, xd, out, out_stride, ntok));
    else if (mt == 2) Q3_TS_SWITCH(w, hipLaunchKernelGGL((k_gemv_kq<LPR, 2, TS>), grid, dim3(64 * nw), 0, st, w, row0, nrows, xq, xd, out, out_stride, ntok));
    else if (mt == 4) Q3_TS_SWITCH(w, hipLaunchKernelGGL((k_gemv_kq<LPR, 4, TS>), grid, dim3(64 * nw), 0, st, w, row0, nrows, xq, xd, out, out_stride, ntok));
    else Q3_TS_SWITCH(w, hipLaunchKernelGGL((k_gemv_kq<LPR, 8, TS>), grid, dim3(64 * nw), 0, st, w, row0, nrows, xq, xd, out, out_stride, ntok));
}

template <int LPR, int MT>
static void gemv_launch(hipStream_t st, const Q8Mat& w, int row0, int nrows, const int8_t* xq, const uint16_t* xd,
                        float* out, int out_stride, int ntok) {
    constexpr int R = 64 / LPR;
    const int nseg = w.K >> 8, nsseg = (nseg + 7) / 8;
    dim3 grid((nrows + R - 1) / R, nsseg, (ntok + MT - 1) / MT);
    const int nw = nseg < 8 ? nseg : 8;
    hipLaunchKernelGGL((k_gemv_q8<LPR, MT>), grid, dim3(64 * nw), 0, st, w, row0, nrows, xq, xd, out, out_stride, ntok);
}
template <int LPR>
static void gemv_launch_mt(hipStream_t st, int mt, const Q8Mat& w, int row0, int nrows, const int8_t* xq, const uint16_t* xd,
                           float* out, int out_stride, int ntok) {
    if (mt == 1) gemv_launch<LPR, 1>(st, w, row0, nrows, xq, xd, out, out_stride, ntok);
    else if (mt == 2) gemv_launch<LPR, 2>(st, w, row0, nrows, xq, xd, out, out_stride, ntok);
    else if (mt == 4) gemv_launch<LPR, 4>(st, w, row0, nrows, xq, xd, out, out_stride, ntok);
    else gemv_launch<LPR, 8>(st, w, row0, nrows, xq, xd, out, out_stride, ntok);
}

static int mt_of(int ntok) { return ntok == 1 ? 1 : ntok == 2 ? 2 : ntok <= 4 ? 4 : 8; }
static int gemv_lpr(long rows32, long rows16) { return rows32 >= 512 ? 2 : rows16 >= 256 ? 4 : 8; }
LinearPlanIn linear_plan_in(int op, const Q8Mat& w, int row0, int nrows, int ntok) {
    LinearPlanIn in;
    in.op = op; in.K = w.K; in.row0 = row0; in.nrows = nrows; in.ntok = ntok;
    in.kq = w.rg_type != nullptr; in.kq_parts = w.nparts; in.wts = wslice_ts(w);
    return in;
}
LinearPlan plan_linear(const LinearPlanIn& in) {
    LinearPlan p;
    const int nseg = in.K >> 8, nsseg = (nseg + 7) / 8, nw = nseg < 8 ? nseg : 8, ntiles = (in.ntok + 31) / 32;
    p.nseg = nseg;
    switch (in.op) {
    case LOP_GEMV: {
        if (in.kq && in.ntok >= 16 && !in.lpr_hint && kq_mfma()) {
            p.form = LIN_GEMM_KQ_MFMA; p.z = mfma_ztiles((in.nrows + 31) / 32, nsseg, in.ntok);
            return p;
        }
        if (in.kq) {
            int lpr = in.lpr_hint;
            if (!lpr) lpr = gemv_lpr((long)(in.nrows / 32) * nsseg, (long)(in.nrows / 16) * nsseg);
            static const bool q6_lpr8 = [] { const char* e = std::getenv("Q3_KQ_Q6_LPR8"); return e && e[0] == '1'; }();
            if (lpr == 8 && !in.lpr_hint && !q6_lpr8 && in.wts != Q3_T_Q5_K && in.wts != Q3_T_Q8_0) lpr = 4;
            p.form = LIN_GEMV_KQ; p.lpr = lpr; p.mt = mt_of(in.ntok);
            return p;
        }
        if (in.ntok >= 16 && !in.lpr_hint) {
            p.z = mfma_ztiles((in.nrows + 31) / 32, nsseg, in.ntok);
            const bool tile1 = p.z == ntiles && nw <= 4 && !(in.nrows & 3) && !(in.out_stride & 3) && !(in.out_addr & 15);
            p.form = tile1 ? LIN_GEMM_Q8_TILE1 : LIN_GEMM_Q8_MFMA;
            return p;
        }
        if (in.ntok > 8 && !in.lpr_hint) { p.form = LIN_GEMM_Q8_TOK; return p; }
        p.form = LIN_GEMV_Q8; p.mt = mt_of(in.ntok);
        p.lpr = in.lpr_hint ? in.lpr_hint : gemv_lpr((long)(in.nrows / 32) * nsseg, (long)(in.nrows / 16) * nsseg);
        return p;
    }
    case LOP_GATEUP: {
        p.form = LIN_GU_UNFUSED;
        if (!in.fused || in.ntok < 16 || (in.K != 1024 && in.K != 2048) || (in.ff & 31)) return p;
        if (in.kq && (!kq_mfma() || in.kq_parts != 1)) return p;
        int z = mfma_ztiles(in.ff / 32, 1, in.ntok);
        if (z < (ntiles + 3) / 4) z = (ntiles + 3) / 4;
        p.z = z;
        p.form = in.kq ? LIN_GU_KQ_MFMA : (z == ntiles && !(in.aq_addr & 3)) ? LIN_GU_Q8_TILE1 : LIN_GU_Q8_MFMA;
        return p;
    }
    case LOP_NORM: p.form = in.ntok > 8 ? LIN_NORM_WG : LIN_NORM; return p;
    case LOP_NORM_GEMV:
        p.form = LIN_GEMV_NORM; p.mt = mt_of(in.ntok);
        p.lpr = in.nrows / 32 >= 512 ? 2 : in.nrows / 16 >= 256 ? 4 : 8;
        return p;
    case LOP_NORM_ARGMAX: p.form = LIN_GEMV_NORM_ARGMAX; p.lpr = 2; p.mt = mt_of(in.ntok); return p;
    case LOP_NORM_GATEUP: p.form = LIN_GU_SWIGLU_NORM; p.mt = in.ntok == 1 ? 1 : in.ntok == 2 ? 2 : 4; return p;
    case LOP_F_GEMV: {
        static const int min_tok = [] { const char* e = std::getenv("Q3_FLOAT_MFMA_MIN"); return e ? atoi(e) : 2; }();
        static const int wide_tok = [] { const char* e = std::getenv("Q3_FLOAT_MFMA_WIDE"); return e ? atoi(e) : 96; }();
        if (!in.has_wt || min_tok <= 0 || in.ntok < min_tok || in.row0 % 64 != 0 || (in.K & 255) != 0 || (in.x_stride & 3) != 0 || (in.x_addr & 15) != 0) {
            p.form = LIN_F_GEMV; p.mt = mt_of(in.ntok);
            return p;
        }
        p.form = in.ntok < wide_tok ? LIN_F_MFMA16 : LIN_F_MFMA;
        return p;
    }
    case LOP_F_GATEUP: {
        static const int max_tok = [] { const char* e = std::getenv("Q3_FLOAT_GU_FUSED_MAX"); return e ? atoi(e) : 95; }();
        const bool ok = in.has_wt && in.ntok >= 2 && in.ntok <= max_tok && in.nrows == 2 * in.ff && (in.ff & 15) == 0 && (in.K & 255) == 0 &&
                        (in.x_stride & 3) == 0 && (in.x_addr & 15) == 0;
        p.form = ok ? LIN_F_GU_MFMA16 : LIN_F_GU_UNFUSED;
        return p;
    }
    default: throw Error("plan_linear: unknown op");
    }
}

void run_gemv_q8(hipStream_t st, const LinearPlan& p, const Q8Mat& w, int row0, int nrows, const int8_t* xq, const uint16_t* xd, float* out,
                 int out_stride, int ntok) {
    const int nseg = w.K >> 8, nsseg = (nseg + 7) / 8, nw = nseg < 8 ? nseg : 8, rgs = (nrows + 31) / 32;
    switch (p.form) {
    case LIN_GEMM_KQ_MFMA:
        Q3_TS_SWITCH(w, hipLaunchKernelGGL((k_gemm_kq_mfma<false, TS>), dim3(rgs, nsseg, p.z), dim3(64 * nw), 0, st, w, row0, nrows, xq, xd, out, out_stride, ntok, 0, (int8_t*)nullptr, (uint16_t*)nullptr));
        return;
    case LIN_GEMV_KQ:
        if (p.lpr == 2) gemv_kq_mt<2>(st, p.mt, w, row0, nrows, xq, xd, out, out_stride, ntok);
        else if (p.lpr == 4) gemv_kq_mt<4>(st, p.mt, w, row0, nrows, xq, xd, out, out_stride, ntok);
        else gemv_kq_mt<8>(st, p.mt, w, row0, nrows, xq, xd, out, out_stride, ntok);
        return;
    case LIN_GEMM_Q8_TILE1:
        hipLaunchKernelGGL((k_gemm_q8_tile1<false>), dim3(rgs, nsseg, p.z), dim3(64 * nw), 0, st, w, row0, nrows, xq, xd, out, out_stride, ntok, 0, (int8_t*)nullptr, (uint16_t*)nullptr);
        return;
    case LIN_GEMM_Q8_MFMA:
        hipLaunchKernelGGL((k_gemm_q8_mfma<false>), dim3(rgs, nsseg, p.z), dim3(64 * nw), 0, st, w, row0, nrows, xq, xd, out, out_stride, ntok, 0, (int8_t*)nullptr, (uint16_t*)nullptr);
        return;
    case LIN_GEMM_Q8_TOK: {
        const size_t lds = 16 * 2048 + 16 * 128 + 8 * 16 * 64 * 4;
        init_kernel_attributes();
        hipLaunchKernelGGL(k_gemm_q8_tok, dim3((nrows + 63) / 64, nsseg, (ntok + 15) / 16), dim3(64 * nw), lds, st, w, row0, nrows, xq, xd, out,
                           out_stride, ntok);
        return;
    }
    case LIN_GEMV_Q8:
        if (p.lpr == 2) gemv_launch_mt<2>(st, p.mt, w, row0, nrows, xq, xd, out, out_stride, ntok);
        else if (p.lpr == 4) gemv_launch_mt<4>(st, p.mt, w, row0, nrows, xq, xd, out, out_stride, ntok);
        else gemv_launch_mt<8>(st, p.mt, w, row0, nrows, xq, xd, out, out_stride, ntok);
        return;
    default: throw Error("run_gemv_q8: not an int8 GEMV form");
    }
}
void launch_gemv_q8(hipStream_t st, const Q8Mat& w, int row0, int nrows, const int8_t* xq, const uint16_t* xd,
                    float* out, int out_stride, int ntok, int lpr_hint) {
    LinearPlanIn in = linear_plan_in(LOP_GEMV, w, row0, nrows, ntok);
    in.out_stride = out_stride; in.out_addr = (uintptr_t)out; in.lpr_hint = lpr_hint;
    run_gemv_q8(st, plan_linear(in), w, row0, nrows, xq, xd, out, out_stride, ntok);
}

void run_gateup_q8(hipStream_t st, const LinearPlan& p, const Q8Mat& wgu, int ff, const int8_t* xq, const uint16_t* xd, int8_t* aq, uint16_t* ad,
                   int ntok) {
    const int rgs = ff / 32;
    if (p.form == LIN_GU_KQ_MFMA)
        Q3_TS_SWITCH(wgu, hipLaunchKernelGGL((k_gemm_kq_mfma<true, TS>), dim3(rgs, 1, p.z), dim3(wgu.K / 4), 0, st, wgu, 0, ff, xq, xd, (float*)nullptr, 0, ntok, ff, aq, ad));
    else if (p.form == LIN_GU_Q8_TILE1) hipLaunchKernelGGL((k_gemm_q8_tile1<true>), dim3(rgs, 1, p.z), dim3(wgu.K / 4), 0, st, wgu, 0, ff, xq, xd, (float*)nullptr, 0, ntok, ff, aq, ad);
    else if (p.form == LIN_GU_Q8_MFMA) hipLaunchKernelGGL((k_gemm_q8_mfma<true>), dim3(rgs, 1, p.z), dim3(wgu.K / 4), 0, st, wgu, 0, ff, xq, xd, (float*)nullptr, 0, ntok, ff, aq, ad);
    else throw Error("run_gateup_q8: not a fused gate/up form");
}
bool launch_gateup_mfma(hipStream_t st, const Q8Mat& wgu, int ff, const int8_t* xq, const uint16_t* xd, int8_t* aq, uint16_t* ad, int ntok) {
    LinearPlanIn in = linear_plan_in(LOP_GATEUP, wgu, 0, 2 * ff, ntok);
    in.ff = ff; in.aq_addr = (uintptr_t)aq;
    const LinearPlan p = plan_linear(in);
    if (p.form == LIN_GU_UNFUSED) return false;
    run_gateup_q8(st, p, wgu, ff, xq, xd, aq, ad, ntok);
    return true;
}

__global__ void __launch_bounds__(512) k_gemm_q8_tok(Q8Mat w, int row0, int nrows, const int8_t* __restrict__ xq,
                                                     const uint16_t* __restrict__ xd, float* __restrict__ out, int out_stride,
                                                     int ntok) {
    constexpr int TT = 16;
    extern __shared__ __attribute__((aligned(16))) unsigned char smem[];
    int8_t* xq_s = reinterpret_cast<int8_t*>(smem);
    uint16_t* xd_s = reinterpret_cast<uint16_t*>(smem + TT * 2048);
    float* red = reinterpret_cast<float*>(smem + TT * 2048 + TT * 128);
    const int lane = threadIdx.x & 63, wave = threadIdx.x >> 6;
    const int nseg = w.K >> 8, nb = w.K >> 5;
    const int sseg = blockIdx.y, seg = sseg * 8 + wave;
    const int tok0 = blockIdx.z * TT;
    int nsg = nseg - sseg * 8;
    if (nsg > 8) nsg = 8;
    const int kspan = nsg * 256;
    const int nt = (ntok - tok0) < TT ? (ntok - tok0) : TT;
    const bool active = seg < nseg;
    uint4 wlo[8], whi[8];
    float dwf[8];
    if (active) {
        int row = row0 + blockIdx.x * 64 + lane;
        if (row > w.Npad - 1) row = w.Npad - 1;
        const int rg = row >> 5, r32 = row & 31;
        const uint8_t* base = w.qs + ((size_t)rg * nb + (size_t)seg * 8) * 1024 + r32 * 16;
#pragma unroll
        for (int i = 0; i < 8; i++) {
            wlo[i] = *reinterpret_cast<const uint4*>(base + (size_t)i * 1024);
            whi[i] = *reinterpret_cast<const uint4*>(base + (size_t)i * 1024 + 512);
        }
        const uint4 dwv = *reinterpret_cast<const uint4*>(w.sc + (((size_t)rg * nseg + seg) * 32 + r32) * 8);
#pragma unroll
        for (int i = 0; i < 8; i++) dwf[i] = h2f(half_of(dwv, i));
    }
    for (int e = threadIdx.x; e < nt * (kspan / 16); e += blockDim.x) {
        const int m = e / (kspan / 16), c = e % (kspan / 16);
        *reinterpret_cast<uint4*>(xq_s + m * 2048 + c * 16) =
            *reinterpret_cast<const uint4*>(xq + (size_t)(tok0 + m) * w.K + sseg * 2048 + c * 16);
    }
    for (int e = threadIdx.x; e < nt * nsg; e += blockDim.x) {
        const int m = e / nsg, c = e % nsg;
        *reinterpret_cast<uint4*>(xd_s + m * 64 + c * 8) = *reinterpret_cast<const uint4*>(xd + (size_t)(tok0 + m) * nb + (sseg * 8 + c) * 8);
    }
    __syncthreads();
    if (active) {
        for (int m = 0; m < nt; m++) {
            const int8_t* xp = xq_s + m * 2048 + wave * 256;
            const uint4 dxv = *reinterpret_cast<const uint4*>(xd_s + m * 64 + wave * 8);
            float acc = 0.0f;
#pragma unroll
            for (int i = 0; i < 8; i++) {
                const uint4 xa = *reinterpret_cast<const uint4*>(xp + i * 32);
                const uint4 xb = *reinterpret_cast<const uint4*>(xp + i * 32 + 16);
                const int isum = dot16(wlo[i], xa) + dot16(whi[i], xb);
                const float sc = dwf[i] * h2f(half_of(dxv, i));
                acc = q3_fmaf((float)isum, sc, acc);
            }
            red[(wave * TT + m) * 64 + lane] = acc;
        }
    }
    __syncthreads();
    for (int t = threadIdx.x; t < nt * 64; t += blockDim.x) {
        const int m = t >> 6, rr = t & 63;
        float S = red[(0 * TT + m) * 64 + rr];
        for (int s = 1; s < nsg; s++) S = S + red[(s * TT + m) * 64 + rr];
        const int orow = blockIdx.x * 64 + rr, tok = tok0 + m;
        if (orow < nrows) out[((size_t)sseg * ntok + tok) * out_stride + orow] = S;
    }
}

#ifndef Q3_GEMM_AB
#define Q3_GEMM_AB 4
#endif
typedef int i32x16 __attribute__((ext_vector_type(16)));
// ... 38 lines not shown
                int atok = tok0 + r;
                if (atok > ntok - 1) atok = ntok - 1;
                const int8_t* xp = xq + (size_t)atok * w.K + seg * 256 + half * 16;
                const uint4 dxa = *reinterpret_cast<const uint4*>(xd + (size_t)atok * nb + seg * 8);
                f32x2v acc2[8];
#pragma unroll
                for (int g = 0; g < 8; g++) acc2[g] = f32x2v{0.0f, 0.0f};
                constexpr int AB = GU ? 2 : Q3_GEMM_AB;
#pragma unroll
                for (int ih = 0; ih < 8 / AB; ih++) {
                    i32x4v av[AB];
#pragma unroll
                    for (int i = 0; i < AB; i++) av[i] = *reinterpret_cast<const i32x4v*>(xp + (AB * ih + i) * 32);
                    f32x32q D;
#pragma unroll
                    for (int i4 = 0; i4 < AB; i4++) {
                        const int i = AB * ih + i4;
                        if ((i4 & 1) == 0) {
#pragma unroll
                            for (int g = 0; g < 32; g++) D[g] = 0.0f;
                            const uint32_t ex = half ? half_of(dxa, i + 1) : half_of(dxa, i), ew = half ? half_of(dwv, i + 1) : half_of(dwv, i);
                            D = __builtin_amdgcn_mfma_f32_32x32x1f32(h2f(ex), h2f(ew), D, 0, 0, 0);
                        }
                        i32x16 c;
#pragma unroll
                        for (int g = 0; g < 16; g++) c[g] = 0;
                        c = __builtin_amdgcn_mfma_i32_32x32x32_i8(av[i4], wv[i], c, 0, 0, 0);
#pragma unroll
                        for (int g4 = 0; g4 < 4; g4++) {
                            const int o = 16 * (i4 & 1) + 4 * g4;
                            const f32x2v sc_a = f32x2v{D[o], D[o + 1]}, sc_b = f32x2v{D[o + 2], D[o + 3]};
                            const f32x2v ca = f32x2v{(float)c[4 * g4], (float)c[4 * g4 + 1]}, cb = f32x2v{(float)c[4 * g4 + 2], (float)c[4 * g4 + 3]};
                            acc2[2 * g4] = __builtin_elementwise_fma(ca, sc_a, acc2[2 * g4]);
                            acc2[2 * g4 + 1] = __builtin_elementwise_fma(cb, sc_b, acc2[2 * g4 + 1]);
                        }
                    }
                }
                if (lt == 0) { if (q == 0) Q3_STAMP_AFTER(1, acc2[7][1]); else Q3_STAMP_AFTER(4, acc2[7][1]); }
#pragma unroll
                for (int g = 0; g < 16; g++) red[wave][(g & 3) + 8 * (g >> 2) + 4 * half][r] = acc2[g >> 1][g & 1];
            }
            wg_barrier_lds();
            if (lt == 0) { if (q == 0) Q3_STAMP(2); else Q3_STAMP(5); }
#pragma unroll 1
            for (int t0 = threadIdx.x; t0 < 32 * 32; t0 += 2 * blockDim.x) {
                float v[2][8];
#pragma unroll
                for (int u = 0; u < 2; u++) {
                    const int t = (t0 + u * (int)blockDim.x) & 1023, m = t >> 5, rr = t & 31;
#pragma unroll
                    for (int s2 = 0; s2 < 8; s2++) v[u][s2] = red[s2][m][rr];
                }
#pragma unroll
                for (int u = 0; u < 2; u++) {
                    const int t = t0 + u * (int)blockDim.x, m = t >> 5, rr = t & 31, tok = tok0 + m;
                    if (t >= 32 * 32) break;
                    float S = v[u][0];
#pragma unroll
                    for (int s2 = 1; s2 < 8; s2++) S = (s2 < nsg) ? S + v[u][s2] : S;
                    if (!GU) {
                        const int orow = blockIdx.x * 32 + rr;
                        if (orow < nrows && tok < ntok) out[((size_t)sseg * ntok + tok) * out_stride + orow] = S;
                    } else if (q == 0) gate_s[lt][t] = S;
                    else {
                        const float y = q3_swiglu(gate_s[lt][t], S);
                        float amax = q3_fabsf(y);
                        amax = fmaxf(amax, xor_lane<16>(amax)); amax = fmaxf(amax, xor_lane<8>(amax)); amax = fmaxf(amax, xor_lane<4>(amax));
                        amax = fmaxf(amax, xor_lane<2>(amax)); amax = fmaxf(amax, xor_lane<1>(amax));
                        const float dd = amax / 127.0f;
                        const float id = (dd != 0.0f) ? (1.0f / dd) : 0.0f;
                        if (tok < ntok) {
                            aq[(size_t)tok * ff + blockIdx.x * 32 + rr] = (int8_t)(int)q3_rintf(y * id);
                            if (rr == 0) ad[(size_t)tok * (ff >> 5) + blockIdx.x] = f2h(dd);
                        }
                    }
                }
            }
            if (q + 1 < NM || tt + (int)gridDim.z < ntiles) wg_barrier_lds();
            if (q == 0 && lt == 0) Q3_STAMP(3);
        }
    }
    Q3_STAMP(6);
    Q3_STAMP_FLUSH();
}


typedef float f32x16q __attribute__((ext_vector_type(16)));
template <bool GU>
__global__ void Q3_GEMM_Q8_BUDGET k_gemm_q8_tile1(Q8Mat w, int row0, int nrows, const int8_t* __restrict__ xq, const uint16_t* __restrict__ xd,
                                                  float* __restrict__ out, int out_stride, int ntok, int ff, int8_t* __restrict__ aq, uint16_t* __restrict__ ad) {
    __shared__ __attribute__((aligned(16))) float red[8][32][36];
    __shared__ __attribute__((aligned(16))) float gate_s[GU ? 1024 : 4];
    const int lane = threadIdx.x & 63, wave = threadIdx.x >> 6;
    const int r = lane & 31, half = lane >> 5;
    const int nseg = w.K >> 8, nb = w.K >> 5;
    const int sseg = blockIdx.y, seg = sseg * 8 + wave;
    int nsg = nseg - sseg * 8;
    if (nsg > 8) nsg = 8;
    const bool active = seg < nseg;
    const int tok0 = blockIdx.z * 32;
    Q3_STAMP_DECL;
    Q3_STAMP(0);
    i32x4v av[8], wv[8];
    uint4 dxa = make_uint4(0, 0, 0, 0), dwv = dxa;
    constexpr int NLATE = GU ? 4 : 0;
    const int8_t* xp = xq;
    auto load_a = [&]() {
        if (!active) return;
        int atok = tok0 + r;
        if (atok > ntok - 1) atok = ntok - 1;
        xp = xq + (size_t)atok * w.K + seg * 256 + half * 16;
        asm volatile("" : "+v"(xp) :: "memory");
#pragma unroll
        for (int i = 0; i < 8 - NLATE; i++) av[i] = *reinterpret_cast<const i32x4v*>(xp + i * 32);
        dxa = *reinterpret_cast<const uint4*>(xd + (size_t)atok * nb + seg * 8);
    };
    load_a();
    auto load_w = [&](int q, int i0, int i1) {
        if (!active) return;
        int row = row0 + blockIdx.x * 32 + r + q * ff;
        if (row > w.Npad - 1) row = w.Npad - 1;
        const int rg = row >> 5, r32 = row & 31;
        const uint8_t* base = w.qs + ((size_t)rg * nb + (size_t)seg * 8) * 1024 + half * 512 + r32 * 16;
        asm volatile("" : "+v"(base) :: "memory");
#pragma unroll
        for (int i = 0; i < 8; i++) if (i >= i0 && i < i1) wv[i] = *reinterpret_cast<const i32x4v*>(base + (size_t)i * 1024);
        if (i0 == 0) dwv = *reinterpret_cast<const uint4*>(w.sc + (((size_t)rg * nseg + seg) * 32 + r32) * 8);
    };
    auto chain = [&]() {
        if (!active) return;
        f32x2v acc2[8];
#pragma unroll
        for (int g = 0; g < 8; g++) acc2[g] = f32x2v{0.0f, 0.0f};
#pragma unroll
        for (int i = 0; i < 8; i++) {
            f32x16q D;
#pragma unroll
            for (int g = 0; g < 16; g++) D[g] = 0.0f;
            const float ex = half ? 0.0f : h2f(half_of(dxa, i)), ew = half ? 0.0f : h2f(half_of(dwv, i));
            D = __builtin_amdgcn_mfma_f32_32x32x2f32(ex, ew, D, 0, 0, 0);
            i32x16 c;
#pragma unroll
            for (int g = 0; g < 16; g++) c[g] = 0;
            c = __builtin_amdgcn_mfma_i32_32x32x32_i8(av[i], wv[i], c, 0, 0, 0);
            if (i < NLATE) {
                const int8_t* xl = xp;
                asm volatile("" : "+v"(xl), "+v"(c) :: "memory");
                av[8 - NLATE + i] = *reinterpret_cast<const i32x4v*>(xl + (8 - NLATE + i) * 32);
            }
#pragma unroll
            for (int g4 = 0; g4 < 4; g4++) {
                const f32x2v sc_a = f32x2v{D[4 * g4], D[4 * g4 + 1]}, sc_b = f32x2v{D[4 * g4 + 2], D[4 * g4 + 3]};
                const f32x2v ca = f32x2v{(float)c[4 * g4], (float)c[4 * g4 + 1]}, cb = f32x2v{(float)c[4 * g4 + 2], (float)c[4 * g4 + 3]};
                acc2[2 * g4] = __builtin_elementwise_fma(ca, sc_a, acc2[2 * g4]);
                acc2[2 * g4 + 1] = __builtin_elementwise_fma(cb, sc_b, acc2[2 * g4 + 1]);
            }
        }
#pragma unroll
        for (int g = 0; g < 16; g++) red[wave][(g & 3) + 8 * (g >> 2) + 4 * half][r] = acc2[g >> 1][g & 1];
    };
    auto seg_sums = [&](int m, int c4) -> float4 {
        float4 v[4];
#pragma unroll
        for (int s2 = 0; s2 < 4; s2++) v[s2] = *reinterpret_cast<const float4*>(&red[s2][m][c4]);
        float4 S = v[0];
#pragma unroll
// ... 993 lines not shown
```

### qwen3-tts-rust_amd/csrc/transformer.h

```cpp
#pragma once
#include "q3_common.h"
#include "gguf.h"
#include "kernels.h"
#include "ggml_mode.h"
#include <memory>

namespace q3 {

struct TfHparams {
    std::string arch;
    int n_embd = 0, n_layer = 0, n_head = 0, n_kv = 0, n_ff = 0, n_vocab = 0;
    float eps = 1e-6f, rope_base = 1e6f;
    int32_t mrope_sec[4] = {0, 0, 0, 0};
};

enum AttnForm { ATTN_UNFUSED = 1, ATTN_FUSED = 2, ATTN_SHORT1 = 3, ATTN_SHORT2 = 4, ATTN_GGML = 5 };
struct AttnPlanIn {
    int ntok = 1;
    bool fused = true; int fused_max_tok = 8;
    bool same_seq = false;
    int short_attn_min = 0;
    int n_head = 1, n_kv = 1;
    int hpw1_max = 128;
    bool float_mode = false, ggml_mode = false;
};
int plan_attention(const AttnPlanIn& in);
void build_rope_tables(float rope_base, int n_ctx, std::vector<float>& cos_out, std::vector<float>& sin_out);

class Transformer {
public:
    Transformer(const std::string& gguf_path, int n_ctx, int max_tok);
    Transformer(const Transformer& weights_of, int max_tok);
    const TfHparams& hp() const { return hp_; }
    int n_ctx() const { return n_ctx_; }
    int max_tok() const { return max_tok_; }
    size_t weight_bytes() const { return weight_bytes_; }
    size_t layer_weight_bytes() const { return layer_weight_bytes_; }
    size_t head_bytes_per_row() const { return (size_t)hp_.n_embd + (size_t)(hp_.n_embd / 32) * 2; }

    struct Input {
        const float* x = nullptr; int x_stride = 0;
        const q3_u64* idx_keys = nullptr; int idx_stride = 0;
        const float* qkv0 = nullptr; int qkv0_stride = 0;
    };
    bool fused = true;
    void forward(hipStream_t st, const Input& in, int ntok, const TokMeta& tm, const KvCache& kv, float* hidden_out);
    void head(hipStream_t st, int tok0, int tok_count, int row0, int nrows, float* logits, int logits_stride,
              const ArgmaxEpi* am = nullptr, int nrows_valid = -1, float* hidden_out = nullptr);
    void build_layer0_qkv(hipStream_t st, const float* x, int x_stride, int64_t rows, float* out);
    void set_same_seq_tokens(bool v) { same_seq_ = v; }
    void set_short_attention(int min_tok, int max_positions) {
        Q3_CHECK(min_tok <= 0 || (max_positions >= 1 && max_positions <= 64), "the short attention form serves at most 64 positions per sequence");
        short_attn_min_ = min_tok;
    }
    void set_fused_max_tokens(int n) { fused_max_tok_ = n; }

    bool ggml_mode() const { return ggml_mode_; }
    int attention_form(int ntok) const;

    LaunchTimer* timer = nullptr;
    LaunchTimer* timer_gu = nullptr;
    const Q8Mat& mat_qkv(int l) const { return layers_[l].wqkv; }
    const Q8Mat& mat_out() const { return output_; }

private:
    void head_impl(hipStream_t st, int tok0, int tok_count, int row0, int nrows, float* logits, int logits_stride, const ArgmaxEpi* am,
                   int nrows_valid, float* hidden_out);
    struct Layer { Q8Mat wqkv, wo, wgu, wdown; FMat fqkv, fo, fgu, fdown; float *attn_norm, *q_norm, *k_norm, *ffn_norm; };
    FMat make_fmat(const Gguf& g, const std::vector<std::string>& names, int K_expect);
    struct Pass { hipStream_t st; int ntok; const TokMeta& tm; const KvCache& kv; int af ; bool fused , wgnorm ; };
    void norm(const Pass& s, const NormPro& a);
    void linear(const Pass& s, const Q8Mat& w, const FMat& fw, const float* xf, const int8_t* xq, const uint16_t* xd, float* out);
    void qkv(const Pass& s, const Layer& L, const NormPro& a);
    void attention(const Pass& s, const Layer& L, int l, const QkvRows& rows);
    void gate_up(const Pass& s, const Layer& L, const NormPro& b);
    bool float_mode_ = false; FMat foutput_; DevBuf<float> xnf_, attf_, actf_;
    float* scratch_logits(int) { return scratch_.p; }
    DevBuf<float> scratch_, hid_, big_logits_;
    void gemv(hipStream_t st, const Q8Mat& w, int row0, int nrows, const int8_t* xq, const uint16_t* xd, float* out,
              int out_stride, int ntok);
    Q8Mat make_mat(const Gguf& g, const std::vector<std::pair<std::string, int>>& rows , int N, int K);
    float* load_f32(const Gguf& g, const std::string& name, int64_t n_expect);
    TfHparams hp_;
    int n_ctx_ = 0, max_tok_ = 0;
    std::vector<Layer> layers_;
    Q8Mat output_;
    float* output_norm_ = nullptr;
    struct WeightStore {
        std::vector<DevBuf<uint8_t>> blobs; DevBuf<float> rope_cos, rope_sin; DevBuf<int32_t> d_mrope;
    };
    std::shared_ptr<WeightStore> ws_;
    std::vector<DevBuf<uint8_t>>& blobs_ = ws_init()->blobs;
    size_t weight_bytes_ = 0, layer_weight_bytes_ = 0;
    DevBuf<float>& rope_cos_ = ws_->rope_cos; DevBuf<float>& rope_sin_ = ws_->rope_sin;
    DevBuf<int32_t>& d_mrope_ = ws_->d_mrope;
    WeightStore* ws_init() { if (!ws_) ws_ = std::make_shared<WeightStore>(); return ws_.get(); }
    void alloc_workspace();
    DevBuf<float> h_, h2_, parts_o_, parts_d_, qkv_, qrot_, gu_;
    bool same_seq_ = false; int short_attn_min_ = 0; int fused_max_tok_ = 8; bool last_fused_ = false; int last_ntok_ = 0;
    DevBuf<int8_t> xq_, aq_, fq_;
    DevBuf<uint16_t> xd_, ad_, fd_;
    int nparts_d_ = 1;
    struct GgLayer { GgMat wq, wk, wv, wo, gate, up, down; };
    bool ggml_mode_ = false;
    std::vector<GgLayer> gg_layers_;
    GgMat gg_output_;
    GgMat gg_load(const Gguf& g, const std::string& name, int n_expect, int k_expect);
    void forward_ggml(hipStream_t st, const Input& in, int ntok, const TokMeta& tm, const KvCache& kv, float* hidden_out);
    void gg_linear(hipStream_t st, const GgMat& w, int row0, int nrows, const float* x, float* out, int out_stride, int ntok);
    GgAct gg_act_{};
    DevBuf<int8_t> gg_q8_, gg_qk_; DevBuf<uint16_t> gg_d8_; DevBuf<float> gg_dk_, gg_xn_, gg_att_, gg_scores_, gg_act_f_; DevBuf<int16_t> gg_bs_;
};

Q8Mat build_q8mat(const WLayout& L, const void* const* raw, DevBuf<uint8_t>& blob);
Q8Mat q8mat_from_host(const void* raw_q8_0, int n, int k, DevBuf<uint8_t>& storage);
Q8Mat kqmat_from_host(const void* const* raw, const int32_t* types, const int32_t* rows, int nw, int k, DevBuf<uint8_t>& storage);

class KvPool {
// ... 26 lines not shown
```

### qwen3-tts-rust_amd/python/q3tts/__init__.py

```python
import ctypes as C
import os
import numpy as np

_HERE = os.path.dirname(os.path.abspath(__file__))
PKG_ROOT = os.path.dirname(os.path.dirname(_HERE))
LIB_PATH = os.path.join(PKG_ROOT, "libq3tts.so")
_lib = None


class Q3Error(RuntimeError):
    pass


class SamplerConfig(C.Structure):
    _fields_ = [("temperature", C.c_float), ("top_k", C.c_int32), ("top_p", C.c_float), ("has_seed", C.c_int32),
                ("seed", C.c_uint64)]


class GenOptions(C.Structure):
    _fields_ = [("repetition_penalty", C.c_float), ("predictor_temperature", C.c_float), ("predictor_top_k", C.c_int32),
                ("predictor_top_p", C.c_float)]


GEN_DEFAULTS = {"repetition_penalty": 1.0, "predictor_temperature": 0.0, "predictor_top_k": 0, "predictor_top_p": 1.0}
# ... 1495 lines not shown
    def summary(self):
        n = lib().q3tts_onnx_summary(self.h, None, 0)
        buf = C.create_string_buffer(n)
        lib().q3tts_onnx_summary(self.h, buf, n)
        return buf.value.decode()

    def node(self, i):
        op, nm = C.c_char_p(), C.c_char_p()
        c = [C.c_int32() for _ in range(3)]
        _chk(lib().q3tts_onnx_node(self.h, i, C.byref(op), C.byref(nm), *[C.byref(x) for x in c]))
        return {"op_type": op.value.decode(), "name": nm.value.decode(),
                "inputs": [lib().q3tts_onnx_node_input(self.h, i, j).decode() for j in range(c[0].value)],
                "outputs": [lib().q3tts_onnx_node_output(self.h, i, j).decode() for j in range(c[1].value)], "n_attr": c[2].value}

    def attr_ints(self, i, name):
        buf = (C.c_int64 * 16)()
        n = lib().q3tts_onnx_node_attr_ints(self.h, i, name.encode(), buf, 16)
        return None if n < 0 else [buf[k] for k in range(min(n, 16))]

    def attr_float(self, i, name):
        f = C.c_float()
        return f.value if lib().q3tts_onnx_node_attr_float(self.h, i, name.encode(), C.byref(f)) == 1 else None

    def initializer(self, i):
        nm, dt, nd, data, nb = C.c_char_p(), C.c_int32(), C.c_int32(), C.c_void_p(), C.c_int64()
        dims = (C.c_int64 * 8)()
        _chk(lib().q3tts_onnx_initializer(self.h, i, C.byref(nm), C.byref(dt), dims, C.byref(nd), C.byref(data), C.byref(nb)))
        raw = C.string_at(data.value, nb.value) if data.value and nb.value else b""
        return {"name": nm.value.decode(), "dtype": dt.value, "dims": [dims[k] for k in range(nd.value)], "raw": raw}

    def decoder_contract(self):
        buf = C.create_string_buffer(4096)
        rc = lib().q3tts_onnx_decoder_contract(self.h, buf, 4096)
        return rc == 0, buf.value.decode()


def onnx_op_kernel(op_type):
    lib().q3tts_onnx_op_kernel.restype = C.c_char_p
    lib().q3tts_onnx_op_kernel.argtypes = [C.c_char_p]
    r = lib().q3tts_onnx_op_kernel(op_type.encode())
    return r.decode() if r else None


class Tokenizer:
    def __init__(self, tokenizer_json):
        L = lib()
        L.q3tts_tokenizer_open.argtypes = [C.c_char_p, C.POINTER(C.c_void_p)]
        L.q3tts_tokenizer_close.argtypes = [C.c_void_p]
        L.q3tts_tokenizer_encode.argtypes = [C.c_void_p, C.c_char_p, C.c_void_p, C.c_int32]
        L.q3tts_tokenizer_decode.restype = C.c_int64
        L.q3tts_tokenizer_decode.argtypes = [C.c_void_p, C.c_void_p, C.c_int32, C.c_char_p, C.c_int64]
        L.q3tts_tokenizer_vocab_size.argtypes = [C.c_void_p]
        h = C.c_void_p()
        _chk(L.q3tts_tokenizer_open(tokenizer_json.encode(), C.byref(h)))
        self.h = h.value

    def close(self):
        if self.h:
            lib().q3tts_tokenizer_close(self.h)
        self.h = None

    def encode(self, text):
        raw = text.encode("utf-8")
        cap = max(16, 2 * len(raw) + 8)
        ids = np.zeros(cap, np.int32)
        n = lib().q3tts_tokenizer_encode(self.h, raw, _p(ids), cap)
        if n < 0:
            raise Q3Error(lib().q3tts_last_error().decode())
        return ids[:n].tolist()

    def decode(self, ids):
        a = np.ascontiguousarray(ids, np.int32)
        n = lib().q3tts_tokenizer_decode(self.h, _p(a), a.size, None, 0)
        if n < 0:
            raise Q3Error(lib().q3tts_last_error().decode())
        buf = C.create_string_buffer(n + 1)
        lib().q3tts_tokenizer_decode(self.h, _p(a), a.size, buf, n + 1)
        return buf.raw[:n].decode("utf-8", errors="replace")


LOP_GEMV, LOP_GATEUP, LOP_NORM, LOP_NORM_GEMV, LOP_NORM_ARGMAX, LOP_NORM_GATEUP, LOP_F_GEMV, LOP_F_GATEUP = range(8)
LIN_FORMS = ["AUTO", "GEMV_Q8", "GEMM_Q8_TOK", "GEMM_Q8_MFMA", "GEMM_Q8_TILE1", "GEMV_KQ", "GEMM_KQ_MFMA", "GU_Q8_TILE1", "GU_Q8_MFMA", "GU_KQ_MFMA",
             "GU_UNFUSED", "NORM", "NORM_WG", "GEMV_NORM", "GEMV_NORM_ARGMAX", "GU_SWIGLU_NORM", "F_GEMV", "F_MFMA16", "F_MFMA", "F_GU_MFMA16",
             "F_GU_UNFUSED"]
LIN = {n: i for i, n in enumerate(LIN_FORMS)}


class LinearDesc(C.Structure):
    _fields_ = [("op", C.c_int32), ("form", C.c_int32),
                ("nw", C.c_int32), ("raw", C.c_void_p * 3), ("type", C.c_int32 * 3), ("rows", C.c_int32 * 3), ("kq_layout", C.c_int32),
                ("K", C.c_int32), ("row0", C.c_int32), ("nrows", C.c_int32), ("nrows_valid", C.c_int32), ("ntok", C.c_int32), ("ff", C.c_int32),
                ("lpr", C.c_int32), ("mt", C.c_int32), ("ztiles", C.c_int32), ("fused", C.c_int32),
                ("xq", C.c_void_p), ("xd", C.c_void_p), ("a_rows", C.c_int32),
                ("x", C.c_void_p), ("x_floats", C.c_int64), ("x_off", C.c_int32), ("x_stride", C.c_int32),
                ("h_in", C.c_void_p), ("h_floats", C.c_int64), ("h_stride", C.c_int32),
                ("idx_keys", C.c_void_p), ("idx", C.c_void_p), ("idx_stride", C.c_int32),
                ("parts", C.c_void_p), ("parts_floats", C.c_int64), ("nparts", C.c_int32), ("parts_stride", C.c_int32), ("parts_slab", C.c_int64),
                ("g", C.c_void_p), ("eps", C.c_float),
                ("h_out", C.c_void_p), ("xn_out", C.c_void_p), ("xq_out", C.c_void_p), ("xd_out", C.c_void_p),
                ("keys", C.c_void_p), ("n_keys", C.c_int64), ("key_stride", C.c_int32), ("mask_per_tok", C.c_void_p), ("idx_add", C.c_int32),
                ("out", C.c_void_p), ("out_floats", C.c_int64), ("out_off", C.c_int64), ("out_stride", C.c_int32),
                ("aq", C.c_void_p), ("ad", C.c_void_p),
                ("form_ran", C.c_int32), ("lpr_ran", C.c_int32), ("mt_ran", C.c_int32), ("z_ran", C.c_int32)]


_LIN_SIZES = {"x": "x_floats", "h_in": "h_floats", "parts": "parts_floats", "out": "out_floats", "keys": "n_keys"}


def _linear_desc(op, form, weights, fields):
    d = LinearDesc()
    d.op = op; d.form = LIN[form] if isinstance(form, str) else form; d.fused = 1
    keep = []
    d.nw = len(weights)
    for i, (raw, t, rows) in enumerate(weights):
        raw = np.ascontiguousarray(raw); keep.append(raw)
        d.raw[i] = raw.ctypes.data if raw.size else None; d.type[i] = t; d.rows[i] = rows
    for k, v in fields.items():
        if isinstance(v, np.ndarray):
            assert v.flags.c_contiguous, k
            keep.append(v)
            setattr(d, k, v.ctypes.data)
            if k in _LIN_SIZES and k + "_n" not in fields:
                setattr(d, _LIN_SIZES[k], v.size)
        elif v is not None:
            setattr(d, k, v)
    return d, keep


def op_linear(op, form="AUTO", weights=(), **fields):
    d, keep = _linear_desc(op, form, list(weights), fields)
    lib().q3tts_op_linear.argtypes = [C.POINTER(LinearDesc)]
    _chk(lib().q3tts_op_linear(C.byref(d)))
    return LIN_FORMS[d.form_ran], d.lpr_ran, d.mt_ran, d.z_ran


def linear_plan(op, weights=(), **fields):
    d, keep = _linear_desc(op, 0, list(weights), fields)
    lib().q3tts_linear_plan.argtypes = [C.POINTER(LinearDesc)]
    _chk(lib().q3tts_linear_plan(C.byref(d)))
    return LIN_FORMS[d.form_ran], d.lpr_ran, d.mt_ran, d.z_ran


def argmax_key(v, idx):
    L = lib()
    L.q3tts_argmax_key.restype = C.c_uint64
    L.q3tts_argmax_key.argtypes = [C.c_float, C.c_int32]
    return int(L.q3tts_argmax_key(v, idx))


SEL_SAMPLE, SEL_SAMPLE_PRED, SEL_ARGMAX, SEL_ARGMAX_KEYS = range(4)
SELECT_SENTINEL = 0xA5C3F00D5A3C0FF1


class SelectDesc(C.Structure):
    _fields_ = [("kernel", C.c_int32), ("B", C.c_int32), ("n", C.c_int32), ("stride", C.c_int32), ("row_off", C.c_int32),
                ("logits", C.c_void_p), ("temperature", C.c_void_p), ("top_k", C.c_void_p), ("top_p", C.c_void_p), ("mask_idx", C.c_void_p),
                ("seed", C.c_void_p), ("draw0", C.c_void_p), ("n_draws", C.c_int32),
                ("penalty", C.c_void_p), ("hist", C.c_void_p), ("hist_len", C.c_void_p), ("hist_cap", C.c_int32), ("cur_code", C.c_void_p),
                ("out_stride", C.c_int32), ("start", C.c_int32), ("end", C.c_int32), ("add", C.c_int32),
                ("tokens", C.c_void_p), ("out_raw", C.c_void_p), ("draws_out", C.c_void_p)]


def select_outputs(B, n_draws=1, out_stride=1):
    return (np.full((n_draws, B), -1, np.int32), np.full((n_draws, B * out_stride), SELECT_SENTINEL, np.uint64),
            np.full(B, 0xFFFFFFFF, np.uint32))


# ... 230 lines not shown
```

Baseline: 728.0.

## Add wide int8 MFMA GEMM forms and enlarge talker prefill chunks to 512

Adds a new int8 MFMA GEMM kernel (plain and fused gate/up with SwiGLU requantisation) that packs four row-group waves into a 256-thread block. The waves share a double-buffered LDS tile of activations and prefetch weights in registers. The planner picks it for quantised Q8 linears with more than 256 tokens. The talker prefill chunk also grows from 256 to 512 when weights are uniform Q8, so prefill runs fewer, larger GEMMs. This is meant to raise activation reuse and MFMA utilisation in prefill, at the cost of more workspace and larger prefill launches that could delay decode steps.

```diff
diff --git a/include/q3tts.h b/include/q3tts.h
--- a/include/q3tts.h
+++ b/include/q3tts.h
@@ -415,7 +415,7 @@
        Q3TTS_LIN_GEMV_KQ = 5, Q3TTS_LIN_GEMM_KQ_MFMA = 6, Q3TTS_LIN_GU_Q8_TILE1 = 7, Q3TTS_LIN_GU_Q8_MFMA = 8, Q3TTS_LIN_GU_KQ_MFMA = 9,
        Q3TTS_LIN_GU_UNFUSED = 10, Q3TTS_LIN_NORM = 11, Q3TTS_LIN_NORM_WG = 12, Q3TTS_LIN_GEMV_NORM = 13, Q3TTS_LIN_GEMV_NORM_ARGMAX = 14,
        Q3TTS_LIN_GU_SWIGLU_NORM = 15, Q3TTS_LIN_F_GEMV = 16, Q3TTS_LIN_F_MFMA16 = 17, Q3TTS_LIN_F_MFMA = 18, Q3TTS_LIN_F_GU_MFMA16 = 19,
-       Q3TTS_LIN_F_GU_UNFUSED = 20 };
+       Q3TTS_LIN_F_GU_UNFUSED = 20, Q3TTS_LIN_GEMM_Q8_WIDE = 21, Q3TTS_LIN_GU_Q8_WIDE = 22 };
 typedef struct q3tts_linear_desc {
     int32_t op, form;
     int32_t nw; const void* raw[3]; int32_t type[3]; int32_t rows[3]; int32_t kq_layout;
diff --git a/qwen3-tts-rust_amd/csrc/capi_ops.cpp b/qwen3-tts-rust_amd/csrc/capi_ops.cpp
--- a/qwen3-tts-rust_amd/csrc/capi_ops.cpp
+++ b/qwen3-tts-rust_amd/csrc/capi_ops.cpp
@@ -149,6 +149,8 @@
 }
 static bool in_set(int v, std::initializer_list<int> s) { for (int x : s) if (v == x) return true; return false; }
 static int op_of_form(int f) {
+    if (f == LIN_GEMM_Q8_WIDE) return LOP_GEMV;
+    if (f == LIN_GU_Q8_WIDE) return LOP_GATEUP;
     if (f <= LIN_GEMM_KQ_MFMA) return LOP_GEMV;
     if (f <= LIN_GU_UNFUSED) return LOP_GATEUP;
     if (f <= LIN_NORM_WG) return LOP_NORM;
@@ -160,7 +162,7 @@
 }
 static void lin_check(const q3tts_linear_desc& d, const LinearPlan& p) {
     const int f = p.form, K = d.K, nt = d.ntok, ntiles = (nt + 31) / 32;
-    Q3_CHECK(f >= LIN_GEMV_Q8 && f <= LIN_F_GU_UNFUSED && op_of_form(f) == d.op, "the form does not compute this op");
+    Q3_CHECK(f >= LIN_GEMV_Q8 && f <= LIN_GU_Q8_WIDE && op_of_form(f) == d.op, "the form does not compute this op");
     const bool quant = lin_quant(d), kq = quant && lin_kq(d), norm = d.op >= LOP_NORM && d.op <= LOP_NORM_GATEUP;
     if (d.op != LOP_NORM) {
         Q3_CHECK(d.nw >= 1 && d.nw <= 3, "1 to 3 weight tensors");
@@ -219,6 +221,11 @@
         Q3_CHECK((K == 1024 || K == 2048) && d.ff % 32 == 0, "fused gate/up: K in {1024, 2048}, ff % 32 == 0");
         Q3_CHECK(p.z >= (ntiles + 3) / 4 && p.z <= ntiles && (f != LIN_GU_Q8_TILE1 || p.z == ntiles), "fused gate/up: ceil(tiles/4) <= ztiles <= tiles (TILE1: == tiles)");
         break;
+    case LIN_GEMM_Q8_WIDE: case LIN_GU_Q8_WIDE:
+        Q3_CHECK(q8, "GEMM_Q8_WIDE / GU_Q8_WIDE take the Q8_0 layout");
+        if (f == LIN_GU_Q8_WIDE) Q3_CHECK((K == 1024 || K == 2048) && d.ff % 32 == 0, "fused gate/up: K in {1024, 2048}, ff % 32 == 0");
+        Q3_CHECK(p.z == ntiles, "wide forms: ztiles == token tiles");
+        break;
     case LIN_GEMV_NORM: case LIN_GEMV_NORM_ARGMAX: case LIN_GU_SWIGLU_NORM:
         Q3_CHECK(f == LIN_GU_SWIGLU_NORM ? (in_set(p.mt, {1, 2, 4}) && lin_wts(d) != -1) : in_set(p.mt, {1, 2, 4, 8}), "mt out of range / GU_SWIGLU_NORM needs one tensor type");
         Q3_CHECK(f == LIN_GU_SWIGLU_NORM || (f == LIN_GEMV_NORM_ARGMAX ? p.lpr == 2 : in_set(p.lpr, {2, 4, 8})), "GEMV_NORM: lpr in {2,4,8}; ARGMAX: lpr 2");
@@ -236,7 +243,7 @@
     q3tts_linear_desc& d = *dp;
     LinearPlan p = lin_plan(d);
     if (d.form != LIN_AUTO) {
-        Q3_CHECK(d.form >= LIN_GEMV_Q8 && d.form <= LIN_F_GU_UNFUSED, "unknown linear form");
+        Q3_CHECK(d.form >= LIN_GEMV_Q8 && d.form <= LIN_GU_Q8_WIDE, "unknown linear form");
         LinearPlan fp; fp.form = d.form; fp.nseg = d.K / 256;
         const int f = d.form, ntiles = (d.ntok + 31) / 32;
         const int mt_def = d.ntok == 1 ? 1 : d.ntok == 2 ? 2 : d.ntok <= 4 ? 4 : 8;
@@ -244,6 +251,7 @@
         fp.lpr = d.lpr ? d.lpr : (p.form == f && p.lpr ? p.lpr : (f == LIN_GEMV_NORM_ARGMAX ? 2 : 8));
         int zdef = p.form == f && p.z ? p.z : ntiles;
         fp.z = d.ztiles ? d.ztiles : zdef;
+        if (f == LIN_GEMM_Q8_WIDE || f == LIN_GU_Q8_WIDE) { fp.mt = 0; fp.lpr = 0; }
         p = fp;
     }
     lin_check(d, p);
@@ -278,14 +286,21 @@
         if (d.xn_out) { dxn.alloc((size_t)nt * K); dxn.upload(d.xn_out, dxn.n); a.xn_out = dxn.p; }
     }
     if (d.out) { dout.alloc((size_t)d.out_floats); dout.upload(d.out, dout.n); }
-    if (d.aq) { daq.alloc((size_t)nt * ff); daq.upload(d.aq, daq.n); dad.alloc((size_t)nt * (ff / 32)); dad.upload(d.ad, dad.n); }
+    constexpr size_t LIN_GUARD = 64;
+    const size_t n_aq = d.aq ? (size_t)nt * ff : 0, n_ad = d.aq ? (size_t)nt * (ff / 32) : 0;
+    if (d.aq) {
+        daq.alloc(n_aq + 2 * LIN_GUARD); dad.alloc(n_ad + 2 * LIN_GUARD);
+        Q3_HIP(hipMemset(daq.p, 0x5A, daq.n)); Q3_HIP(hipMemset(dad.p, 0x5A, dad.n * 2));
+        Q3_HIP(hipMemcpy(daq.p + LIN_GUARD, d.aq, n_aq, hipMemcpyHostToDevice)); Q3_HIP(hipMemcpy(dad.p + LIN_GUARD, d.ad, n_ad * 2, hipMemcpyHostToDevice));
+    }
+    int8_t* const aqp = d.aq ? daq.p + LIN_GUARD : nullptr; uint16_t* const adp = d.aq ? dad.p + LIN_GUARD : nullptr;
     float* out = d.out ? dout.p + d.out_off : nullptr;
     switch (p.form) {
-    case LIN_GEMV_Q8: case LIN_GEMM_Q8_TOK: case LIN_GEMM_Q8_MFMA: case LIN_GEMM_Q8_TILE1: case LIN_GEMV_KQ: case LIN_GEMM_KQ_MFMA:
+    case LIN_GEMV_Q8: case LIN_GEMM_Q8_TOK: case LIN_GEMM_Q8_MFMA: case LIN_GEMM_Q8_TILE1: case LIN_GEMV_KQ: case LIN_GEMM_KQ_MFMA: case LIN_GEMM_Q8_WIDE:
         run_gemv_q8(0, p, m, d.row0, d.nrows, dxq.p, dxd.p, out, d.out_stride, nt);
         break;
-    case LIN_GU_Q8_TILE1: case LIN_GU_Q8_MFMA: case LIN_GU_KQ_MFMA:
-        run_gateup_q8(0, p, m, ff, dxq.p, dxd.p, daq.p, dad.p, nt);
+    case LIN_GU_Q8_TILE1: case LIN_GU_Q8_MFMA: case LIN_GU_KQ_MFMA: case LIN_GU_Q8_WIDE:
+        run_gateup_q8(0, p, m, ff, dxq.p, dxd.p, aqp, adp, nt);
         break;
     case LIN_GU_UNFUSED: {
         dgu.alloc((size_t)((K / 256 + 7) / 8) * nt * 2 * ff);
@@ -293,7 +308,7 @@
         gi.out_stride = 2 * ff; gi.out_addr = (uintptr_t)dgu.p;
         const LinearPlan gp = plan_linear(gi);
         run_gemv_q8(0, gp, m, 0, 2 * ff, dxq.p, dxd.p, dgu.p, 2 * ff, nt);
-        launch_swiglu_quant(0, dgu.p, ff, daq.p, dad.p, nt);
+        launch_swiglu_quant(0, dgu.p, ff, aqp, adp, nt);
         p.lpr = gp.lpr; p.mt = gp.mt; p.z = gp.z;
         break;
     }
@@ -316,7 +331,7 @@
         } else run_gemv_q8_norm(0, p, m, d.row0, d.nrows, a, out, d.out_stride, nt, nullptr);
         break;
     }
-    case LIN_GU_SWIGLU_NORM: run_gateup_swiglu(0, p, m, ff, a, daq.p, dad.p, nt); break;
+    case LIN_GU_SWIGLU_NORM: run_gateup_swiglu(0, p, m, ff, a, aqp, adp, nt); break;
     case LIN_F_GEMV: case LIN_F_MFMA16: case LIN_F_MFMA:
         run_gemv_float(0, p, fm, d.row0, d.nrows, dx.p + d.x_off, d.x_stride, out, d.out_stride, nt);
         break;
@@ -342,7 +357,13 @@
     if (p.form == LIN_F_GU_MFMA16) Q3_HIP(hipMemcpy2D(out, (size_t)d.out_stride * 4, dgu.p, (size_t)ff * 4, (size_t)ff * 4, nt, hipMemcpyDeviceToDevice));
     Q3_HIP(hipDeviceSynchronize());
     if (d.out) dout.download(d.out, dout.n);
-    if (d.aq) { daq.download(d.aq, daq.n); dad.download(d.ad, dad.n); }
+    if (d.aq) {
+        std::vector<int8_t> hq(daq.n); std::vector<uint16_t> hd(dad.n);
+        daq.download(hq.data(), hq.size()); dad.download(hd.data(), hd.size());
+        for (size_t i = 0; i < LIN_GUARD; i++)
+            Q3_CHECK(hq[i] == 0x5A && hq[LIN_GUARD + n_aq + i] == 0x5A && hd[i] == 0x5A5A && hd[LIN_GUARD + n_ad + i] == 0x5A5A, "gate/up form wrote outside aq / ad");
+        std::memcpy(d.aq, hq.data() + LIN_GUARD, n_aq); std::memcpy(d.ad, hd.data() + LIN_GUARD, n_ad * 2);
+    }
     if (d.h_out) dhout.download(d.h_out, dhout.n);
     if (d.xn_out) dxn.download(d.xn_out, dxn.n);
     if (dxq_out.p) { dxq_out.download(d.xq_out, dxq_out.n); dxd_out.download(d.xd_out, dxd_out.n); }
diff --git a/qwen3-tts-rust_amd/csrc/engine.cpp b/qwen3-tts-rust_amd/csrc/engine.cpp
--- a/qwen3-tts-rust_amd/csrc/engine.cpp
+++ b/qwen3-tts-rust_amd/csrc/engine.cpp
@@ -28,6 +28,7 @@
     const int B = p.max_batch;
     B_ = B;
     talker_.reset(new Transformer(dir + "/qwen3_tts_talker.gguf", Q3_TALKER_NCTX, std::max(256, B)));
+    if (talker_->q8_uniform() && prefill_wide()) { pf_chunk_ = 512; if (talker_->max_tok() < pf_chunk_) talker_->set_max_tok(pf_chunk_); }
     predictor_.reset(new Transformer(dir + "/qwen3_tts_predictor.gguf", Q3_PRED_NCTX, 2 * B));
     if (const char* e = std::getenv("Q3_PRED_FUSED_MAX")) predictor_->set_fused_max_tokens(atoi(e));
     {
@@ -85,10 +86,10 @@
         async_pf_ = B > 1 && !(e && e[0] == '0');
     }
     if (async_pf_) {
-        talker_pf_.reset(new Transformer(*talker_, 256));
+        talker_pf_.reset(new Transformer(*talker_, pf_chunk_));
         Q3_HIP(hipStreamCreateWithFlags(&st_pf_, hipStreamNonBlocking));
         Q3_HIP(hipEventCreate(&pf_done_)); Q3_HIP(hipEventCreate(&pf_e0_));
-        lane_alloc(pf_, talker_pf_.get(), st_pf_, 256, true, (size_t)4096 * (Q3_EMBD * 4 + 24 + 68 + 64) + ((size_t)1 << 16) + (size_t)B * 4);
+        lane_alloc(pf_, talker_pf_.get(), st_pf_, pf_chunk_, true,(size_t)4096 * (Q3_EMBD * 4 + 24 + 68 + 64) + ((size_t)1 << 16) + (size_t)B * 4);
     }
     hist_stride_ = p.max_steps * 16;
     tl_stride_ = (Q3_SAMPLE_END + 31) & ~31;
@@ -1106,7 +1107,7 @@
     Q3_HIP(hipGetDevice(&prev));
     Q3_HIP(hipSetDevice(dev_));
     try {
-        const int W = score_w_, rows = std::max(talker_->max_tok(), 256);
+        const int W = score_w_, rows = std::max(talker_->max_tok(), pf_chunk_);
         pred_sc_.reset(new Transformer(*predictor_, 16 * W));
         kv_sc_.reset(new KvPool(predictor_->hp().n_layer, predictor_->hp().n_kv, W, W, 1));
         for (int w = 0; w < W; w++) kv_sc_->ensure(w, 16);
diff --git a/qwen3-tts-rust_amd/csrc/engine.h b/qwen3-tts-rust_amd/csrc/engine.h
--- a/qwen3-tts-rust_amd/csrc/engine.h
+++ b/qwen3-tts-rust_amd/csrc/engine.h
@@ -181,6 +181,7 @@
     hipStream_t st_pf_ = nullptr; PrefillLane ar_, pf_;
     DevBuf<float> d_pf_logits_, d_pf_hidden_;
     std::vector<Req*> pf_batch_; hipEvent_t pf_done_ = nullptr, pf_e0_ = nullptr; bool async_pf_ = false; int n_prefilling_ = 0;
+    int pf_chunk_ = 256;
     std::unique_ptr<KvPool> kv_t_, kv_p_;
     std::unique_ptr<CodecDecoder> codec_;
     DevBuf<float> d_codec_tab_[16]; DevBuf<float> d_proj_tab_[16];
diff --git a/qwen3-tts-rust_amd/csrc/kernels.h b/qwen3-tts-rust_amd/csrc/kernels.h
--- a/qwen3-tts-rust_amd/csrc/kernels.h
+++ b/qwen3-tts-rust_amd/csrc/kernels.h
@@ -147,7 +147,8 @@
 enum LinearForm { LIN_AUTO = 0, LIN_GEMV_Q8 = 1, LIN_GEMM_Q8_TOK = 2, LIN_GEMM_Q8_MFMA = 3, LIN_GEMM_Q8_TILE1 = 4, LIN_GEMV_KQ = 5,
                   LIN_GEMM_KQ_MFMA = 6, LIN_GU_Q8_TILE1 = 7, LIN_GU_Q8_MFMA = 8, LIN_GU_KQ_MFMA = 9, LIN_GU_UNFUSED = 10, LIN_NORM = 11,
                   LIN_NORM_WG = 12, LIN_GEMV_NORM = 13, LIN_GEMV_NORM_ARGMAX = 14, LIN_GU_SWIGLU_NORM = 15, LIN_F_GEMV = 16, LIN_F_MFMA16 = 17,
-                  LIN_F_MFMA = 18, LIN_F_GU_MFMA16 = 19, LIN_F_GU_UNFUSED = 20 };
+                  LIN_F_MFMA = 18, LIN_F_GU_MFMA16 = 19, LIN_F_GU_UNFUSED = 20, LIN_GEMM_Q8_WIDE = 21, LIN_GU_Q8_WIDE = 22 };
+bool prefill_wide();
 struct LinearPlanIn {
     int op = LOP_GEMV;
     int K = 0, row0 = 0, nrows = 0, ntok = 0, ff = 0;
diff --git a/qwen3-tts-rust_amd/csrc/kernels.hip b/qwen3-tts-rust_amd/csrc/kernels.hip
--- a/qwen3-tts-rust_amd/csrc/kernels.hip
+++ b/qwen3-tts-rust_amd/csrc/kernels.hip
@@ -82,6 +82,10 @@
                                float* __restrict__ out, int out_stride, int ntok, int ff, int8_t* __restrict__ aq, uint16_t* __restrict__ ad);
 template <bool GU>
 __global__ void Q3_GEMM_Q8_BUDGET k_gemm_q8_tile1(Q8Mat w, int row0, int nrows, const int8_t* __restrict__ xq, const uint16_t* __restrict__ xd,
+                               float* __restrict__ out, int out_stride, int ntok, int ff, int8_t* __restrict__ aq, uint16_t* __restrict__ ad);
+#define Q3_GEMM_Q8_WIDE_BUDGET __launch_bounds__(256) __attribute__((amdgpu_waves_per_eu(2, 2)))
+template <bool GU>
+__global__ void Q3_GEMM_Q8_WIDE_BUDGET k_gemm_q8_wide(Q8Mat w, int row0, int nrows, const int8_t* __restrict__ xq, const uint16_t* __restrict__ xd,
                                float* __restrict__ out, int out_stride, int ntok, int ff, int8_t* __restrict__ aq, uint16_t* __restrict__ ad);
 template <int TYPE>
 __global__ void __launch_bounds__(512) __attribute__((amdgpu_waves_per_eu(2, 2)))
@@ -111,6 +115,7 @@
     int z = (target + rowgroups * nsseg - 1) / (rowgroups * nsseg);
     return z < 1 ? 1 : (z > ntiles ? ntiles : z);
 }
+bool prefill_wide() { const char* e = std::getenv("Q3_PREFILL_WIDE"); return !(e && e[0] == '0'); }
 
 template <int LPR, int MT, int TS>
 __global__ void __launch_bounds__(512) k_gemv_kq(Q8Mat w, int row0, int nrows, const int8_t* __restrict__ xq,
@@ -217,6 +222,10 @@
             p.form = LIN_GEMV_KQ; p.lpr = lpr; p.mt = mt_of(in.ntok);
             return p;
         }
+        if (in.ntok > 256 && !in.lpr_hint && prefill_wide()) {
+            p.form = LIN_GEMM_Q8_WIDE; p.z = ntiles;
+            return p;
+        }
         if (in.ntok >= 16 && !in.lpr_hint) {
             p.z = mfma_ztiles((in.nrows + 31) / 32, nsseg, in.ntok);
             const bool tile1 = p.z == ntiles && nw <= 4 && !(in.nrows & 3) && !(in.out_stride & 3) && !(in.out_addr & 15);
@@ -232,6 +241,10 @@
         p.form = LIN_GU_UNFUSED;
         if (!in.fused || in.ntok < 16 || (in.K != 1024 && in.K != 2048) || (in.ff & 31)) return p;
         if (in.kq && (!kq_mfma() || in.kq_parts != 1)) return p;
+        if (!in.kq && in.ntok > 256 && prefill_wide()) {
+            p.form = LIN_GU_Q8_WIDE; p.z = ntiles;
+            return p;
+        }
         int z = mfma_ztiles(in.ff / 32, 1, in.ntok);
         if (z < (ntiles + 3) / 4) z = (ntiles + 3) / 4;
         p.z = z;
@@ -284,6 +297,10 @@
     case LIN_GEMM_Q8_MFMA:
         hipLaunchKernelGGL((k_gemm_q8_mfma<false>), dim3(rgs, nsseg, p.z), dim3(64 * nw), 0, st, w, row0, nrows, xq, xd, out, out_stride, ntok, 0, (int8_t*)nullptr, (uint16_t*)nullptr);
         return;
+    case LIN_GEMM_Q8_WIDE:
+        if ((uint64_t)w.Npad * w.K >= (1ull << 32) || (uint64_t)ntok * w.K >= (1ull << 32)) throw Error("GEMM_Q8_WIDE: 32-bit lane offsets (matrix and activations below 4 GiB)");
+        hipLaunchKernelGGL((k_gemm_q8_wide<false>), dim3((rgs + 3) / 4, nsseg, (ntok + 31) / 32), dim3(256), 0, st, w, row0, nrows, xq, xd, out, out_stride, ntok, 0, (int8_t*)nullptr, (uint16_t*)nullptr);
+        return;
     case LIN_GEMM_Q8_TOK: {
         const size_t lds = 16 * 2048 + 16 * 128 + 8 * 16 * 64 * 4;
         init_kernel_attributes();
@@ -313,7 +330,10 @@
         Q3_TS_SWITCH(wgu, hipLaunchKernelGGL((k_gemm_kq_mfma<true, TS>), dim3(rgs, 1, p.z), dim3(wgu.K / 4), 0, st, wgu, 0, ff, xq, xd, (float*)nullptr, 0, ntok, ff, aq, ad));
     else if (p.form == LIN_GU_Q8_TILE1) hipLaunchKernelGGL((k_gemm_q8_tile1<true>), dim3(rgs, 1, p.z), dim3(wgu.K / 4), 0, st, wgu, 0, ff, xq, xd, (float*)nullptr, 0, ntok, ff, aq, ad);
     else if (p.form == LIN_GU_Q8_MFMA) hipLaunchKernelGGL((k_gemm_q8_mfma<true>), dim3(rgs, 1, p.z), dim3(wgu.K / 4), 0, st, wgu, 0, ff, xq, xd, (float*)nullptr, 0, ntok, ff, aq, ad);
-    else throw Error("run_gateup_q8: not a fused gate/up form");
+    else if (p.form == LIN_GU_Q8_WIDE) {
+        if ((uint64_t)wgu.Npad * wgu.K >= (1ull << 32) || (uint64_t)ntok * wgu.K >= (1ull << 32)) throw Error("GU_Q8_WIDE: 32-bit lane offsets (matrix and activations below 4 GiB)");
+        hipLaunchKernelGGL((k_gemm_q8_wide<true>), dim3((rgs + 3) / 4, 1, (ntok + 31) / 32), dim3(256), 0, st, wgu, 0, ff, xq, xd, (float*)nullptr, 0, ntok, ff, aq, ad);
+    } else throw Error("run_gateup_q8: not a fused gate/up form");
 }
 bool launch_gateup_mfma(hipStream_t st, const Q8Mat& wgu, int ff, const int8_t* xq, const uint16_t* xd, int8_t* aq, uint16_t* ad, int ntok) {
     LinearPlanIn in = linear_plan_in(LOP_GATEUP, wgu, 0, 2 * ff, ntok);
@@ -518,6 +538,179 @@
     }
     Q3_STAMP(6);
     Q3_STAMP_FLUSH();
+}
+
+template <bool GU>
+__global__ void Q3_GEMM_Q8_WIDE_BUDGET k_gemm_q8_wide(Q8Mat w, int row0, int nrows, const int8_t* __restrict__ xq, const uint16_t* __restrict__ xd,
+                                                      float* __restrict__ out, int out_stride, int ntok, int ff, int8_t* __restrict__ aq,
+                                                      uint16_t* __restrict__ ad) {
+    constexpr int T = 1, TT = 32 * T, NQ = GU ? 2 : 1, NA = NQ * T;
+    constexpr int XROW = 272;
+    constexpr int PF = 8 / NQ;
+    constexpr int NP = 2 * T, PSTEP = 4 / NP;
+    __shared__ __attribute__((aligned(16))) unsigned char xs[2][TT * XROW];
+    __shared__ __attribute__((aligned(16))) uint4 ds[2][TT];
+    const int lane = threadIdx.x & 63, wave = threadIdx.x >> 6;
+    const int r = lane & 31, half = lane >> 5;
+    const int nseg = w.K >> 8, nb = w.K >> 5;
+    const int sseg = blockIdx.y;
+    int nsg = nseg - sseg * 8;
+    if (nsg > 8) nsg = 8;
+    const int nblk = nsg * 8;
+    const int tok0 = blockIdx.z * TT;
+    const int rgi = blockIdx.x * 4 + wave;
+    const bool active = rgi * 32 < nrows;
+    const int pc = threadIdx.x & 15, pm = threadIdx.x >> 4;
+    uint32_t xoff[NP];
+#pragma unroll
+    for (int k = 0; k < NP; k++) {
+        int tok = tok0 + pm + 16 * k;
+        if (tok > ntok - 1) tok = ntok - 1;
+        xoff[k] = (uint32_t)tok * (uint32_t)w.K + pc * 16;
+    }
+    const int8_t* const xseg0 = xq + (size_t)sseg * 2048;
+    auto xaddr = [&](int k, int s) { return reinterpret_cast<const uint4*>(xseg0 + (size_t)s * 256 + xoff[k]); };
+    const int dm = threadIdx.x % TT;
+    int dtok = tok0 + dm;
+    if (dtok > ntok - 1) dtok = ntok - 1;
+    const uint32_t doff = (uint32_t)dtok * (uint32_t)nb;
+    const uint16_t* const dseg0 = xd + sseg * 64;
+    auto daddr = [&](int s) { return reinterpret_cast<const uint4*>(dseg0 + (size_t)s * 8 + doff); };
+    uint32_t woff[NQ], scoff[NQ];
+#pragma unroll
+    for (int q = 0; q < NQ; q++) {
+        int row = row0 + rgi * 32 + r + q * ff;
+        if (row > w.Npad - 1) row = w.Npad - 1;
+        const int rg = row >> 5, r32 = row & 31;
+        woff[q] = ((uint32_t)rg * (uint32_t)nb) * 1024u + half * 512 + r32 * 16;
+        scoff[q] = (((uint32_t)rg * (uint32_t)nseg) * 32 + r32) * 8 + half;
+    }
+    const uint8_t* const wseg0 = w.qs + (size_t)sseg * 64 * 1024;
+    const uint16_t* const scseg0 = w.sc + (size_t)sseg * 8 * 256;
+    auto waddr = [&](int q, int blk) { return reinterpret_cast<const i32x4v*>(wseg0 + (size_t)blk * 1024 + woff[q]); };
+    auto scaddr = [&](int q, int pair) { return scseg0 + (size_t)((pair >> 2) * 256 + (pair & 3) * 2) + scoff[q]; };
+    i32x4v wv[NQ][PF];
+    uint32_t ew[NQ];
+#pragma unroll
+    for (int q = 0; q < NQ; q++) {
+#pragma unroll
+        for (int i = 0; i < PF; i++) wv[q][i] = *waddr(q, i);
+        ew[q] = *scaddr(q, 0);
+    }
+#pragma unroll
+    for (int k = 0; k < NP; k++) *reinterpret_cast<uint4*>(&xs[0][(pm + 16 * k) * XROW + pc * 16]) = *xaddr(k, 0);
+    ds[0][dm] = *daddr(0);
+    wg_barrier_lds();
+    f32x2v acc2[NA][8], S2[NA][8];
+    i32x16 cmagic;
+#pragma unroll
+    for (int g = 0; g < 16; g++) cmagic[g] = 0x4B400000;
+    asm volatile("" : "+v"(cmagic));
+    const f32x2v fmagic = f32x2v{12582912.0f, 12582912.0f};
+#pragma unroll 1
+    for (int s = 0; s < nsg; s++) {
+        const int p = s & 1;
+        const bool more = s + 1 < nsg;
+#pragma unroll
+        for (int a = 0; a < NA; a++)
+#pragma unroll
+            for (int g = 0; g < 8; g++) acc2[a][g] = f32x2v{0.0f, 0.0f};
+#pragma unroll
+        for (int ip = 0; ip < 4; ip++) {
+            const bool stage = ip % PSTEP == 0;
+            const int k = ip / PSTEP;
+            const int sn = more ? s + 1 : s;
+            uint4 px = make_uint4(0, 0, 0, 0), pd = px;
+            if (stage) px = *xaddr(k, sn);
+            if (stage && k == 0) pd = *daddr(sn);
+            uint32_t ewn[NQ];
+            {
+                int lp = s * 4 + ip + 1;
+                if (lp > nsg * 4 - 1) lp = nsg * 4 - 1;
+#pragma unroll
+                for (int q = 0; q < NQ; q++) ewn[q] = *scaddr(q, lp);
+            }
+            __builtin_amdgcn_sched_barrier(0);
+#pragma unroll
+            for (int j = 0; j < T; j++) {
+                const unsigned char* xp = &xs[p][(j * 32 + r) * XROW + half * 16 + ip * 64];
+                const i32x4v av0 = *reinterpret_cast<const i32x4v*>(xp), av1 = *reinterpret_cast<const i32x4v*>(xp + 32);
+                const uint32_t ex = reinterpret_cast<const uint16_t*>(&ds[p][j * 32 + r])[2 * ip + half];
+#pragma unroll
+                for (int q = 0; q < NQ; q++) {
+                    const int a = q * T + j;
+                    f32x32q D;
+#pragma unroll
+                    for (int g = 0; g < 32; g++) D[g] = 0.0f;
+                    D = __builtin_amdgcn_mfma_f32_32x32x1f32(h2f(ex), h2f(ew[q]), D, 0, 0, 0);
+#pragma unroll
+                    for (int i2 = 0; i2 < 2; i2++) {
+                        const i32x16 c = __builtin_amdgcn_mfma_i32_32x32x32_i8(i2 ? av1 : av0, wv[q][(2 * ip + i2) % PF], cmagic, 0, 0, 0);
+#pragma unroll
+                        for (int g4 = 0; g4 < 4; g4++) {
+                            const int o = 16 * i2 + 4 * g4;
+                            const f32x2v sc_a = f32x2v{D[o], D[o + 1]}, sc_b = f32x2v{D[o + 2], D[o + 3]};
+                            const f32x2v ca = f32x2v{__int_as_float(c[4 * g4]), __int_as_float(c[4 * g4 + 1])} - fmagic;
+                            const f32x2v cb = f32x2v{__int_as_float(c[4 * g4 + 2]), __int_as_float(c[4 * g4 + 3])} - fmagic;
+                            acc2[a][2 * g4] = __builtin_elementwise_fma(ca, sc_a, acc2[a][2 * g4]);
+                            acc2[a][2 * g4 + 1] = __builtin_elementwise_fma(cb, sc_b, acc2[a][2 * g4 + 1]);
+                        }
+                        asm volatile("" : "+v"(acc2[a][0]), "+v"(acc2[a][1]), "+v"(acc2[a][2]), "+v"(acc2[a][3]), "+v"(acc2[a][4]), "+v"(acc2[a][5]),
+                                          "+v"(acc2[a][6]), "+v"(acc2[a][7]));
+                    }
+                    __builtin_amdgcn_sched_barrier(0);
+                }
+            }
+            if (stage) *reinterpret_cast<uint4*>(&xs[p ^ 1][(pm + 16 * k) * XROW + pc * 16]) = px;
+            if (stage && k == 0) ds[p ^ 1][dm] = pd;
+#pragma unroll
+            for (int q = 0; q < NQ; q++) {
+#pragma unroll
+                for (int i2 = 0; i2 < 2; i2++) {
+                    int nxt = s * 8 + 2 * ip + i2 + PF;
+                    if (nxt > nblk - 1) nxt = nblk - 1;
+                    wv[q][(2 * ip + i2) % PF] = *waddr(q, nxt);
+                }
+                ew[q] = ewn[q];
+            }
+            __builtin_amdgcn_sched_barrier(0);
+        }
+        if (s == 0) {
+#pragma unroll
+            for (int a = 0; a < NA; a++)
+#pragma unroll
+                for (int g = 0; g < 8; g++) S2[a][g] = acc2[a][g];
+        } else {
+#pragma unroll
+            for (int a = 0; a < NA; a++)
+#pragma unroll
+                for (int g = 0; g < 8; g++) S2[a][g] = S2[a][g] + acc2[a][g];
+        }
+        if (more) wg_barrier_lds();
+    }
+    if (!active) return;
+#pragma unroll
+    for (int j = 0; j < T; j++) {
+#pragma unroll
+        for (int g = 0; g < 16; g++) {
+            const int tok = tok0 + j * 32 + (g & 3) + 8 * (g >> 2) + 4 * half;
+            if (!GU) {
+                const int orow = rgi * 32 + r;
+                if (orow < nrows && tok < ntok) out[((size_t)sseg * ntok + tok) * out_stride + orow] = S2[j][g >> 1][g & 1];
+            } else {
+                const float y = q3_swiglu(S2[j][g >> 1][g & 1], S2[T + j][g >> 1][g & 1]);
+                float amax = q3_fabsf(y);
+                amax = fmaxf(amax, xor_lane<16>(amax)); amax = fmaxf(amax, xor_lane<8>(amax)); amax = fmaxf(amax, xor_lane<4>(amax));
+                amax = fmaxf(amax, xor_lane<2>(amax)); amax = fmaxf(amax, xor_lane<1>(amax));
+                const float dd = amax / 127.0f;
+                const float id = (dd != 0.0f) ? (1.0f / dd) : 0.0f;
+                if (tok < ntok) {
+                    aq[(size_t)tok * ff + rgi * 32 + r] = (int8_t)(int)q3_rintf(y * id);
+                    if (r == 0) ad[(size_t)tok * (ff >> 5) + rgi] = f2h(dd);
+                }
+            }
+        }
+    }
 }
 
 
diff --git a/qwen3-tts-rust_amd/csrc/transformer.h b/qwen3-tts-rust_amd/csrc/transformer.h
--- a/qwen3-tts-rust_amd/csrc/transformer.h
+++ b/qwen3-tts-rust_amd/csrc/transformer.h
@@ -34,6 +34,12 @@
     const TfHparams& hp() const { return hp_; }
     int n_ctx() const { return n_ctx_; }
     int max_tok() const { return max_tok_; }
+    void set_max_tok(int max_tok) { max_tok_ = max_tok; alloc_workspace(); }
+    bool q8_uniform() const {
+        if (float_mode_ || ggml_mode_) return false;
+        for (const Layer& L : layers_) if (L.wqkv.rg_type || L.wo.rg_type || L.wgu.rg_type || L.wdown.rg_type) return false;
+        return true;
+    }
     size_t weight_bytes() const { return weight_bytes_; }
     size_t layer_weight_bytes() const { return layer_weight_bytes_; }
     size_t head_bytes_per_row() const { return (size_t)hp_.n_embd + (size_t)(hp_.n_embd / 32) * 2; }
diff --git a/qwen3-tts-rust_amd/python/q3tts/__init__.py b/qwen3-tts-rust_amd/python/q3tts/__init__.py
--- a/qwen3-tts-rust_amd/python/q3tts/__init__.py
+++ b/qwen3-tts-rust_amd/python/q3tts/__init__.py
@@ -1601,7 +1601,7 @@
 LOP_GEMV, LOP_GATEUP, LOP_NORM, LOP_NORM_GEMV, LOP_NORM_ARGMAX, LOP_NORM_GATEUP, LOP_F_GEMV, LOP_F_GATEUP = range(8)
 LIN_FORMS = ["AUTO", "GEMV_Q8", "GEMM_Q8_TOK", "GEMM_Q8_MFMA", "GEMM_Q8_TILE1", "GEMV_KQ", "GEMM_KQ_MFMA", "GU_Q8_TILE1", "GU_Q8_MFMA", "GU_KQ_MFMA",
              "GU_UNFUSED", "NORM", "NORM_WG", "GEMV_NORM", "GEMV_NORM_ARGMAX", "GU_SWIGLU_NORM", "F_GEMV", "F_MFMA16", "F_MFMA", "F_GU_MFMA16",
-             "F_GU_UNFUSED"]
+             "F_GU_UNFUSED", "GEMM_Q8_WIDE", "GU_Q8_WIDE"]
 LIN = {n: i for i, n in enumerate(LIN_FORMS)}
 
 
```

New measurement: 742.4 (median of 6 runs). 1.02x the previous value.
